# bartn8/vppstereo

Hardware: AMD Instinct MI355X
Metric: Mdisparities/s (HxWxD / s) VPP+rSGM at 540x960xD=192 (higher is better)
Workload: dtype u16

## Files before the change

### include/vppx.h

```cpp
#ifndef VPPX_H
#define VPPX_H

#include <stddef.h>
#include <stdint.h>

#ifdef __cplusplus
extern "C" {
#endif

#define VPPX_VERSION 100

enum {
    VPPX_OK = 0,
    VPPX_E_INVALID_ARG = -1,
    VPPX_E_DMAX_MOD8 = -2,
    VPPX_E_DMAX_GT256 = -3,
    VPPX_E_UNIQUENESS = -4,
    VPPX_E_WIDTH_MOD16 = -5,
    VPPX_E_METHOD = -6,
    VPPX_E_NO_DEVICE = -7,
    VPPX_E_HIP = -8,
    VPPX_E_OOM = -9,
    VPPX_E_UNSUPPORTED = -10
};
// ... 217 lines not shown
typedef struct vppx_fstream vppx_fstream;
int vppx_fstream_create(vppx_ctx *ctx, const VppxOccParams *op, const VppxVppParams *vp, const VppxRsgmParams *rp, int batch,
                        int depth, int H, int W, int C, int flags, int copy_threads, vppx_fstream **out);
void vppx_fstream_destroy(vppx_fstream *fs);
int vppx_fstream_create_scaled(vppx_ctx *ctx, const VppxOccParams *op, const VppxVppParams *vp, const VppxRsgmParams *rp,
                               const VppxScaleParams *sp, int batch, int depth, int H, int W, int C, int flags, int copy_threads,
                               vppx_fstream **out);

int vppx_fstream_push(vppx_fstream *fs, const uint8_t *left, const uint8_t *right, const float *hints, const uint8_t *g_occ);
int vppx_fstream_push_guided(vppx_fstream *fs, const uint8_t *left, const uint8_t *right, const float *hints, const uint8_t *g_occ,
                             const float *validhints);
int vppx_fstream_flush(vppx_fstream *fs);
int vppx_fstream_pop(vppx_fstream *fs, float *disp_out, uint8_t *l_vpp_out, uint8_t *r_vpp_out, uint8_t *conf_out,
                     uint64_t *draws_out, int *got);
int vppx_fstream_create_eval(vppx_ctx *ctx, const VppxOccParams *op, const VppxVppParams *vp, const VppxRsgmParams *rp,
                             const VppxScaleParams *sp, const VppxEvalParams *ep, int batch, int depth, int H, int W, int C, int flags,
                             int copy_threads, vppx_fstream **out);
int vppx_fstream_push_eval(vppx_fstream *fs, const uint8_t *left, const uint8_t *right, const float *hints, const uint8_t *g_occ,
                           const float *validhints, const float *gt, const float *validgt);
int vppx_fstream_pop_eval(vppx_fstream *fs, float *disp_out, uint8_t *l_vpp_out, uint8_t *r_vpp_out, uint8_t *conf_out,
                          uint64_t *draws_out, VppxMetrics *metrics_out, int *got);
int vppx_fstream_create_sampled(vppx_ctx *ctx, const VppxOccParams *op, const VppxVppParams *vp, const VppxRsgmParams *rp,
                                const VppxScaleParams *sp, const VppxEvalParams *ep, const VppxSampleParams *smp, int batch, int depth,
                                int H, int W, int C, int flags, int copy_threads, vppx_fstream **out);
int vppx_fstream_push_sampled(vppx_fstream *fs, const uint8_t *left, const uint8_t *right, const uint8_t *g_occ, const float *src,
                              const float *validsrc, const float *gt, const float *validgt);
int vppx_fstream_counts(vppx_fstream *fs, int64_t *pushed, int64_t *filling, int64_t *unpopped, int64_t *reruns);

int vppx_u8_to_nchw_dev(vppx_ctx *ctx, int B, int H, int W, int C, int pad_multiple, const uint8_t *src, void *dst,
                        int dst_is_bf16);

int vppx_psmnet_cost_volume_dev(vppx_ctx *ctx, const float *fea_l, const float *fea_r, const float *hints,
                                const float *validhints, int B, int C, int H4, int W4, int H, int W, int maxdisp,
                                float *cost);
int vppx_raft_corr_modulate_dev(vppx_ctx *ctx, float *corr, const float *hints, const float *validhints, int B, int H4,
                                int W2, int W3, int H, int W);
typedef enum VppxDtype {
    VPPX_DT_F32 = 0,
    VPPX_DT_BF16 = 1
} VppxDtype;
int vppx_psmnet_cost_volume_dt_dev(vppx_ctx *ctx, const void *fea_l, const void *fea_r, const float *hints,
                                   const float *validhints, int B, int C, int H4, int W4, int H, int W, int maxdisp,
                                   void *cost, int dtype);
int vppx_raft_corr_modulate_dt_dev(vppx_ctx *ctx, void *corr, const float *hints, const float *validhints, int B, int H4,
                                   int W2, int W3, int H, int W, int dtype);
#define VPPX_CORR_MAX_LEVELS 4
#define VPPX_CORR_MAX_RADIUS 8
int64_t vppx_raft_corr_pyramid_cells(int64_t N, int W3, int levels, int64_t *offsets);
int vppx_raft_corr_pyramid_dt_dev(vppx_ctx *ctx, void *corr, const float *hints, const float *validhints, int B, int H4, int W2,
                                  int W3, int H, int W, int levels, void *pyr, int dtype);
int vppx_raft_corr_lookup_dt_dev(vppx_ctx *ctx, const void *corr, const void *pyr, const float *coords_x,
                                 int64_t coords_frame_stride, int B, int H4, int W2, int W3, int levels, int radius,
                                 float *out, int dtype);
int vppx_psmnet_readout_dt_dev(vppx_ctx *ctx, const void *cost, int B, int D4, int H4, int W4, int maxdisp, int H, int W,
                               int top, int left, int Hout, int Wout, float *out, int dtype);
int vppx_raft_upsample_dt_dev(vppx_ctx *ctx, const void *flow, int64_t flow_frame_stride, const void *mask, int B, int C,
                              int H4, int W4, int f, int mask_channels, int sign, int top, int left, int Hout, int Wout,
                              float *out, int dtype);
int vppx_kitti_disp_decode_dev(vppx_ctx *ctx, const uint16_t *png_u16, int64_t n, float *disp, uint8_t *valid);
int vppx_png_decode_dev(vppx_ctx *ctx, int n_files, const uint8_t *blob, const int64_t *offsets, int H, int W, int C,
                        float scale, float *disp, uint8_t *valid, uint8_t *out_u8, int32_t *status);
int vppx_pfm_decode_dev(vppx_ctx *ctx, const uint8_t *raw, int H, int W, int channels, int little_endian, float *out);

int vppx_occlusion_heuristic_host(vppx_ctx *ctx, int B, int H, int W, const float *hints, int rx, int ry, double l,
                                  double g, double th_conf, double th_filter, uint8_t *conf_out);
int vppx_occlusion_heuristic_dev(vppx_ctx *ctx, int B, int H, int W, const float *hints, int rx, int ry, double l,
                                 double g, double th_conf, double th_filter, uint8_t *conf_out);
int vppx_occlusion_heuristic_full_host(vppx_ctx *ctx, int B, int H, int W, const float *hints, int rx, int ry, double l,
                                       double g, double th_conf, double th_filter, float *dmap_out, uint8_t *conf_out);
int vppx_occlusion_heuristic_full_dev(vppx_ctx *ctx, int B, int H, int W, const float *hints, int rx, int ry, double l,
                                      double g, double th_conf, double th_filter, float *dmap_out, uint8_t *conf_out);

int vppx_set_graph_mode(vppx_ctx *ctx, int enable);
long vppx_graph_replays(vppx_ctx *ctx);
int vppx_time_aggregate(vppx_ctx *ctx, int iters, float *ms_out);
int vppx_agg_kernel_ms(vppx_ctx *ctx, int last_n, float *avg_ms, int *n_used);
int vppx_we_kernel_ms(vppx_ctx *ctx, int last_n, float *avg_ms, int *n_used);
int vppx_time_aggregate_frames(vppx_ctx *ctx);
int vppx_time_aggregate_part(vppx_ctx *ctx, int iters, int part, float *ms_out);
int vppx_uses_vert(vppx_ctx *ctx);
int vppx_fused_pixels_per_wave(vppx_ctx *ctx);
int vppx_batch_quantum(vppx_ctx *ctx, int H, int W, int dmax);
int vppx_last_call_parts(vppx_ctx *ctx);
int vppx_we_last_pieces(vppx_ctx *ctx);
int vppx_wsum_last_pieces(vppx_ctx *ctx);
int vppx_wsum_default_route(int B, int Hp, int Wp, int dmax, int p2max, int nsimd);
int vppx_last_routes(vppx_ctx *ctx, char *buf, int n);
int vppx_last_front_routes(vppx_ctx *ctx, char *buf, int n);
int vppx_enable_stage_timing(vppx_ctx *ctx, int enable);
int vppx_get_stage_ms(vppx_ctx *ctx, float *ms, int max_n);
const char *vppx_stage_name(int i);


#ifdef __cplusplus
}
#endif
#endif
```

### vppstereo_amd/_lib.py

```python
import ctypes as C
import os
import threading

import numpy as np

_HERE = os.path.dirname(os.path.abspath(__file__))
LIB_PATH = os.environ.get("VPPX_LIB") or os.path.join(_HERE, "libvppx.so")

VPPX_OK = 0
ERR_NAMES = {
    -1: "VPPX_E_INVALID_ARG", -2: "VPPX_E_DMAX_MOD8", -3: "VPPX_E_DMAX_GT256", -4: "VPPX_E_UNIQUENESS",
    -5: "VPPX_E_WIDTH_MOD16", -6: "VPPX_E_METHOD", -7: "VPPX_E_NO_DEVICE", -8: "VPPX_E_HIP", -9: "VPPX_E_OOM",
    -10: "VPPX_E_UNSUPPORTED",
}

EXPORTS = [
    "vppx_version", "vppx_last_error", "vppx_vpp_params_default", "vppx_rsgm_params_default", "vppx_occ_params_default", "vppx_create",
    "vppx_destroy", "vppx_set_stream", "vppx_set_stream_legacy", "vppx_set_pipeline", "vppx_synchronize", "vppx_status", "vppx_lockstep_failures", "vppx_workspace_bytes", "vppx_device_name", "vppx_srand",
    "vppx_rand_stream", "vppx_rand_state", "vppx_rand_advance", "vppx_virtual_projection_scan_rnd", "vppx_virtual_projection_scan_max_dist", "vppx_vpp_host",
    "vppx_vpp_dev", "vppx_vpp_last_draws", "vppx_census5x5", "vppx_cost_census5x5_xyd", "vppx_aggregate", "vppx_aggregate_img", "vppx_match_wta",
    "vppx_match_wta_right", "vppx_subpixel_refine", "vppx_median3x3", "vppx_rsgm_host", "vppx_rsgm_dev",
    "vppx_vpp_rsgm_dev", "vppx_rsgm_post_dev", "vppx_occ_vpp_rsgm_dev", "vppx_occ_vpp_rsgm_host", "vppx_inputs_ready_event", "vppx_u8_to_nchw_dev", "vppx_psmnet_cost_volume_dev", "vppx_raft_corr_modulate_dev", "vppx_kitti_disp_decode_dev", "vppx_png_decode_dev", "vppx_pfm_decode_dev", "vppx_occlusion_heuristic_host", "vppx_occlusion_heuristic_dev", "vppx_occlusion_heuristic_full_host", "vppx_occlusion_heuristic_full_dev", "vppx_set_graph_mode", "vppx_graph_replays", "vppx_time_aggregate", "vppx_agg_kernel_ms", "vppx_we_kernel_ms", "vppx_time_aggregate_frames", "vppx_time_aggregate_part", "vppx_uses_vert", "vppx_last_call_parts", "vppx_we_last_pieces", "vppx_wsum_last_pieces", "vppx_wsum_default_route", "vppx_last_routes", "vppx_last_front_routes", "vppx_fused_pixels_per_wave", "vppx_batch_quantum",
    "vppx_enable_stage_timing", "vppx_get_stage_ms", "vppx_stage_name",
    "vppx_fstream_create", "vppx_fstream_destroy", "vppx_fstream_push", "vppx_fstream_flush", "vppx_fstream_pop", "vppx_fstream_counts",
    "vppx_occ_vpp_rsgm_guided_dev", "vppx_occ_vpp_rsgm_guided_host", "vppx_fstream_push_guided",
    "vppx_scale_params_default", "vppx_scaled_shape", "vppx_scale_table_builds", "vppx_last_front_sets", "vppx_occ_vpp_rsgm_scaled_dev", "vppx_occ_vpp_rsgm_scaled_host",
    "vppx_fstream_create_scaled",
    "vppx_eval_params_default", "vppx_guided_metrics_dev", "vppx_guided_metrics_host", "vppx_occ_vpp_rsgm_eval_dev",
    "vppx_fstream_create_eval", "vppx_fstream_push_eval", "vppx_fstream_pop_eval",
    "vppx_rsgm_front_dev", "vppx_rsgm_guided_rows_dev", "vppx_rsgm_mid_dev",
    "vppx_error_colors_dev", "vppx_error_colors_host", "vppx_guided_visualize_dev", "vppx_guided_visualize_host",
    "vppx_colorize_dev", "vppx_colorize_host", "vppx_finite_max_dev",
    "vppx_sample_params_default", "vppx_sample_threshold", "vppx_sample_hints_dev", "vppx_sample_hints_host", "vppx_occ_vpp_rsgm_sampled_dev",
    "vppx_fstream_create_sampled", "vppx_fstream_push_sampled",
    "vppx_psmnet_cost_volume_dt_dev", "vppx_raft_corr_modulate_dt_dev",
    "vppx_raft_corr_pyramid_cells", "vppx_raft_corr_pyramid_dt_dev", "vppx_raft_corr_lookup_dt_dev",
    "vppx_psmnet_readout_dt_dev", "vppx_raft_upsample_dt_dev",
]
CORR_MAX_LEVELS, CORR_MAX_RADIUS = 4, 8
DT_F32, DT_BF16 = 0, 1
FS_PATTERNS, FS_MASK, FS_GOCC, FS_GUIDED = 1, 2, 4, 8
FS_METRICS, FS_NO_DISP = 16, 32
FS_SAMPLE = 64
VIZ_KEYS = ('bad 1.0', 'bad 2.0', 'bad 3.0', 'bad 4.0', 'avgerr', 'rms')
VIZ_ALL = 63
VIZ_MAX_DILATION = 31
METRIC_KEYS = ('bad 1.0', 'bad 2.0', 'bad 3.0', 'bad 4.0', 'avgerr', 'rms')


class VppxVppParams(C.Structure):
    _fields_ = [
        ("method", C.c_int32), ("wsize", C.c_int32), ("wsize_agg_x", C.c_int32), ("wsize_agg_y", C.c_int32),
        ("direction", C.c_int32), ("uniform_color", C.c_int32), ("discard_occluded", C.c_int32),
        ("interpolate", C.c_int32), ("c", C.c_float), ("c_occ", C.c_float), ("use_distance_patch", C.c_int32),
        ("use_bilateral_patch", C.c_int32), ("distance_gamma", C.c_double), ("dmin", C.c_float), ("dmax", C.c_float),
        ("seed", C.c_uint32), ("per_frame_range", C.c_uint32), ("rand_offset", C.c_uint64),
        ("bilateral_o_xy", C.c_double), ("bilateral_o_i", C.c_double), ("bilateral_th", C.c_double),
    ]


class VppxRsgmParams(C.Structure):
    _fields_ = [
        ("dmax", C.c_int32), ("p1", C.c_int32), ("p2min", C.c_int32), ("alpha", C.c_float), ("gamma", C.c_int32),
        ("uniqueness", C.c_float), ("subpixel", C.c_int32), ("reserved0", C.c_int32),
    ]


class VppxOccParams(C.Structure):
    _fields_ = [("rx", C.c_int32), ("ry", C.c_int32), ("l", C.c_double), ("g", C.c_double), ("th_conf", C.c_double),
                ("th_filter", C.c_double)]


class VppxScaleParams(C.Structure):
    _fields_ = [("iscale", C.c_int32), ("oscale", C.c_int32)]


class VppxEvalParams(C.Structure):
    _fields_ = [("gt_scale", C.c_int32), ("reserved0", C.c_int32)]


class VppxSampleParams(C.Structure):
    _fields_ = [("probability", C.c_double), ("seed", C.c_uint32), ("reserved0", C.c_uint32), ("reserved1", C.c_uint64)]


class VppxMetrics(C.Structure):
    _fields_ = [("bad1", C.c_double), ("bad2", C.c_double), ("bad3", C.c_double), ("bad4", C.c_double), ("avgerr", C.c_double),
                ("rms", C.c_double), ("n_valid", C.c_double), ("reserved", C.c_double)]


class VppxError(Exception):

    def __init__(self, code, msg):
        super().__init__(msg)
        self.code = code


_lib = None
_lock = threading.Lock()


def load():
    global _lib
    with _lock:
        if _lib is not None:
            return _lib
# ... 13 lines not shown
        lib.vppx_device_name.restype = C.c_char_p
        lib.vppx_device_name.argtypes = [vp]
        lib.vppx_stage_name.restype = C.c_char_p
        lib.vppx_stage_name.argtypes = [C.c_int]
        lib.vppx_workspace_bytes.restype = C.c_size_t
        lib.vppx_workspace_bytes.argtypes = [vp]
        lib.vppx_create.argtypes = [C.POINTER(vp), C.c_int]
        lib.vppx_destroy.argtypes = [vp]
        lib.vppx_destroy.restype = None
        lib.vppx_set_stream.argtypes = [vp, vp]
        lib.vppx_set_stream_legacy.argtypes = [vp]
        lib.vppx_set_pipeline.argtypes = [vp, C.c_int]
        lib.vppx_synchronize.argtypes = [vp]
        lib.vppx_status.argtypes = [vp]
        lib.vppx_lockstep_failures.argtypes = [vp]
        lib.vppx_lockstep_failures.restype = C.c_long
        lib.vppx_srand.argtypes = [vp, C.c_uint32]
        lib.vppx_rand_state.argtypes = [vp, C.POINTER(C.c_uint32), C.POINTER(C.c_uint64)]
        lib.vppx_rand_advance.argtypes = [vp, C.c_uint64]
        lib.vppx_rand_stream.argtypes = [vp, C.c_uint32, C.c_uint64, C.c_int64, vp]
        i, f, d = C.c_int, C.c_float, C.c_double
        lib.vppx_virtual_projection_scan_rnd.argtypes = [vp, vp, vp, vp, i, i, i, i, i, i, f, f, vp, i, i]
        lib.vppx_virtual_projection_scan_max_dist.argtypes = [vp, vp, vp, vp, i, i, i, i, i, i, i, i, f, f, vp, i, i]
        pv, pr = C.POINTER(VppxVppParams), C.POINTER(VppxRsgmParams)
        lib.vppx_vpp_params_default.argtypes = [pv]
        lib.vppx_vpp_params_default.restype = None
        lib.vppx_rsgm_params_default.argtypes = [pr]
        lib.vppx_rsgm_params_default.restype = None
        lib.vppx_vpp_host.argtypes = [vp, pv, i, i, i, i, vp, vp, vp, vp, vp, vp]
        lib.vppx_vpp_dev.argtypes = [vp, pv, i, i, i, i, vp, vp, vp, vp, vp, vp]
        lib.vppx_vpp_last_draws.argtypes = [vp, i, C.POINTER(C.c_uint64)]
        lib.vppx_census5x5.argtypes = [vp, vp, vp, i, i]
        lib.vppx_cost_census5x5_xyd.argtypes = [vp, vp, vp, vp, i, i, i, i]
        lib.vppx_aggregate.argtypes = [vp, vp, vp, vp, i, i, i, i, i, f, i]
        lib.vppx_aggregate_img.argtypes = [vp, vp, i, vp, vp, i, i, i, i, i, f, i]
        lib.vppx_match_wta.argtypes = [vp, vp, vp, i, i, i, f]
        lib.vppx_match_wta_right.argtypes = [vp, vp, vp, i, i, i, f]
        lib.vppx_subpixel_refine.argtypes = [vp, vp, vp, i, i, i, i]
        lib.vppx_median3x3.argtypes = [vp, vp, vp, i, i]
        lib.vppx_rsgm_host.argtypes = [vp, pr, i, i, i, i, vp, vp, vp, vp, vp, vp]
        lib.vppx_rsgm_dev.argtypes = [vp, pr, i, i, i, i, vp, vp, vp, vp, vp, vp]
        lib.vppx_rsgm_post_dev.argtypes = [vp, i, i, i, vp, vp, i, vp]
        lib.vppx_rsgm_front_dev.argtypes = [vp, i, i, i, i, vp, vp, vp, vp, vp, vp]
        lib.vppx_rsgm_guided_rows_dev.argtypes = [vp, i, i, i, i, vp, vp, vp, vp, vp, vp, vp]
        lib.vppx_rsgm_mid_dev.argtypes = [vp, i, i, i, vp, vp, vp, vp]
        lib.vppx_vpp_rsgm_dev.argtypes = [vp, pv, pr, i, i, i, i, vp, vp, vp, vp, vp, vp, vp]
        po = C.POINTER(VppxOccParams)
        lib.vppx_occ_vpp_rsgm_host.argtypes = [vp, po, pv, pr, i, i, i, i, vp, vp, vp, vp, vp, vp, vp, vp, C.POINTER(C.c_uint64)]
        lib.vppx_occ_params_default.argtypes = [po]
        lib.vppx_occ_params_default.restype = None
        lib.vppx_occ_vpp_rsgm_dev.argtypes = [vp, po, pv, pr, i, i, i, i, vp, vp, vp, vp, vp, vp, vp]
        lib.vppx_occ_vpp_rsgm_guided_dev.argtypes = [vp, po, pv, pr, i, i, i, i, vp, vp, vp, vp, vp, vp, vp, vp, vp]
        lib.vppx_occ_vpp_rsgm_guided_host.argtypes = [vp, po, pv, pr, i, i, i, i, vp, vp, vp, vp, vp, vp, vp, vp, vp,
                                                      C.POINTER(C.c_uint64)]
        lib.vppx_inputs_ready_event.argtypes = [vp, vp]
        lib.vppx_u8_to_nchw_dev.argtypes = [vp, i, i, i, i, i, vp, vp, i]
        lib.vppx_psmnet_cost_volume_dev.argtypes = [vp, vp, vp, vp, vp, i, i, i, i, i, i, i, vp]
        lib.vppx_raft_corr_modulate_dev.argtypes = [vp, vp, vp, vp, i, i, i, i, i, i]
        lib.vppx_psmnet_cost_volume_dt_dev.argtypes = [vp, vp, vp, vp, vp, i, i, i, i, i, i, i, vp, i]
        lib.vppx_raft_corr_modulate_dt_dev.argtypes = [vp, vp, vp, vp, i, i, i, i, i, i, i]
        lib.vppx_raft_corr_pyramid_cells.argtypes = [C.c_int64, i, i, C.POINTER(C.c_int64)]
        lib.vppx_raft_corr_pyramid_cells.restype = C.c_int64
        lib.vppx_raft_corr_pyramid_dt_dev.argtypes = [vp, vp, vp, vp, i, i, i, i, i, i, i, vp, i]
        lib.vppx_raft_corr_lookup_dt_dev.argtypes = [vp, vp, vp, vp, C.c_int64, i, i, i, i, i, i, vp, i]
        lib.vppx_psmnet_readout_dt_dev.argtypes = [vp, vp, i, i, i, i, i, i, i, i, i, i, i, vp, i]
        lib.vppx_raft_upsample_dt_dev.argtypes = [vp, vp, C.c_int64, vp, i, i, i, i, i, i, i, i, i, i, i, vp, i]
        lib.vppx_kitti_disp_decode_dev.argtypes = [vp, vp, C.c_int64, vp, vp]
        lib.vppx_pfm_decode_dev.argtypes = [vp, vp, i, i, i, i, vp]
        lib.vppx_png_decode_dev.argtypes = [vp, i, vp, C.POINTER(C.c_int64), i, i, i, f, vp, vp, vp, vp]
        lib.vppx_occlusion_heuristic_host.argtypes = [vp, i, i, i, vp, i, i, d, d, d, d, vp]
        lib.vppx_occlusion_heuristic_dev.argtypes = [vp, i, i, i, vp, i, i, d, d, d, d, vp]
        lib.vppx_occlusion_heuristic_full_host.argtypes = [vp, i, i, i, vp, i, i, d, d, d, d, vp, vp]
        lib.vppx_occlusion_heuristic_full_dev.argtypes = [vp, i, i, i, vp, i, i, d, d, d, d, vp, vp]
        lib.vppx_set_graph_mode.argtypes = [vp, i]
        lib.vppx_graph_replays.argtypes = [vp]
        lib.vppx_graph_replays.restype = C.c_long
        lib.vppx_time_aggregate.argtypes = [vp, i, C.POINTER(C.c_float)]
        lib.vppx_agg_kernel_ms.argtypes = [vp, i, C.POINTER(C.c_float), C.POINTER(C.c_int)]
        lib.vppx_we_kernel_ms.argtypes = [vp, i, C.POINTER(C.c_float), C.POINTER(C.c_int)]
        lib.vppx_time_aggregate_frames.argtypes = [vp]
        lib.vppx_time_aggregate_part.argtypes = [vp, i, i, C.POINTER(C.c_float)]
        lib.vppx_uses_vert.argtypes = [vp]
        lib.vppx_last_call_parts.argtypes = [vp]
        lib.vppx_we_last_pieces.argtypes = [vp]
        lib.vppx_wsum_last_pieces.argtypes = [vp]
        lib.vppx_wsum_default_route.argtypes = [i, i, i, i, i, i]
        lib.vppx_last_routes.argtypes = [vp, C.c_char_p, i]
        lib.vppx_last_front_routes.argtypes = [vp, C.c_char_p, i]
        lib.vppx_fused_pixels_per_wave.argtypes = [vp]
        lib.vppx_batch_quantum.argtypes = [vp, i, i, i]
        lib.vppx_enable_stage_timing.argtypes = [vp, i]
        lib.vppx_get_stage_ms.argtypes = [vp, C.POINTER(C.c_float), i]
        lib.vppx_fstream_create.argtypes = [vp, po, pv, pr, i, i, i, i, i, i, i, C.POINTER(vp)]
        lib.vppx_fstream_destroy.argtypes = [vp]
        lib.vppx_fstream_destroy.restype = None
        lib.vppx_fstream_push.argtypes = [vp, vp, vp, vp, vp]
        lib.vppx_fstream_push_guided.argtypes = [vp, vp, vp, vp, vp, vp]
        lib.vppx_fstream_flush.argtypes = [vp]
        lib.vppx_fstream_pop.argtypes = [vp, vp, vp, vp, vp, C.POINTER(C.c_uint64), C.POINTER(C.c_int)]
        ps = C.POINTER(VppxScaleParams)
        lib.vppx_scale_params_default.argtypes = [ps]
        lib.vppx_scale_params_default.restype = None
        pi = C.POINTER(C.c_int)
        lib.vppx_scaled_shape.argtypes = [i, i, ps, pi, pi, pi, pi]
        lib.vppx_scale_table_builds.argtypes = [vp]
        lib.vppx_scale_table_builds.restype = C.c_long
        lib.vppx_last_front_sets.argtypes = [vp, pi, pi]
        lib.vppx_occ_vpp_rsgm_scaled_dev.argtypes = [vp, po, pv, pr, ps, i, i, i, i, vp, vp, vp, vp, vp, vp, vp, vp, vp, vp]
        lib.vppx_occ_vpp_rsgm_scaled_host.argtypes = [vp, po, pv, pr, ps, i, i, i, i, vp, vp, vp, vp, vp, vp, vp, vp, vp, vp,
                                                      C.POINTER(C.c_uint64)]
        lib.vppx_fstream_create_scaled.argtypes = [vp, po, pv, pr, ps, i, i, i, i, i, i, i, C.POINTER(vp)]
        p64 = C.POINTER(C.c_int64)
        lib.vppx_fstream_counts.argtypes = [vp, p64, p64, p64, p64]
        pe = C.POINTER(VppxEvalParams)
        lib.vppx_eval_params_default.argtypes = [pe]
        lib.vppx_eval_params_default.restype = None
        lib.vppx_guided_metrics_dev.argtypes = [vp, pe, i, i, i, vp, i, i, vp, vp, vp, vp]
        lib.vppx_guided_metrics_host.argtypes = [vp, pe, i, i, i, vp, i, i, vp, vp, vp, vp]
        lib.vppx_occ_vpp_rsgm_eval_dev.argtypes = [vp, po, pv, pr, ps, pe, i, i, i, i, vp, vp, vp, vp, vp, vp, vp, vp, vp, vp, vp, vp, vp, vp]
        lib.vppx_fstream_create_eval.argtypes = [vp, po, pv, pr, ps, pe, i, i, i, i, i, i, i, C.POINTER(vp)]
        lib.vppx_fstream_push_eval.argtypes = [vp, vp, vp, vp, vp, vp, vp, vp]
        lib.vppx_fstream_pop_eval.argtypes = [vp, vp, vp, vp, vp, C.POINTER(C.c_uint64), C.POINTER(VppxMetrics), C.POINTER(C.c_int)]
        u = C.c_uint
        for sfx in ("dev", "host"):
            getattr(lib, "vppx_error_colors_" + sfx).argtypes = [vp, i, i, i, vp, vp, d, i, i, vp]
            getattr(lib, "vppx_guided_visualize_" + sfx).argtypes = [vp, i, i, i, vp, vp, vp, d, i, u, vp]
            getattr(lib, "vppx_colorize_" + sfx).argtypes = [vp, i, i, i, vp, vp, vp, i, vp]
        lib.vppx_finite_max_dev.argtypes = [vp, i, i, i, vp, vp]
        pm = C.POINTER(VppxSampleParams)
        lib.vppx_sample_params_default.argtypes = [pm]
        lib.vppx_sample_params_default.restype = None
        lib.vppx_sample_threshold.argtypes = [d]
        lib.vppx_sample_threshold.restype = C.c_uint32
        lib.vppx_sample_hints_dev.argtypes = [vp, pm, i, i, i, vp, vp, vp, vp]
        lib.vppx_sample_hints_host.argtypes = [vp, pm, i, i, i, vp, vp, vp, vp]
        lib.vppx_occ_vpp_rsgm_sampled_dev.argtypes = [vp, po, pv, pr, ps, pe, pm, i, i, i, i, vp, vp, vp, vp, i, vp, vp, vp, vp, vp, vp, vp, vp,
                                                      vp, vp, vp, vp]
        lib.vppx_fstream_create_sampled.argtypes = [vp, po, pv, pr, ps, pe, pm, i, i, i, i, i, i, i, C.POINTER(vp)]
        lib.vppx_fstream_push_sampled.argtypes = [vp, vp, vp, vp, vp, vp, vp, vp]
        _lib = lib
        return lib


def split_routes(s):
    out, depth, cur = [], 0, []
    for ch in s:
        if ch == "," and depth == 0:
            out.append("".join(cur))
            cur = []
            continue
        depth += (ch == "<") - (ch == ">")
        cur.append(ch)
    if cur:
        out.append("".join(cur))
    return out


def _route_list(fn, handle):
    n = check(fn(handle, None, 0))
    buf = C.create_string_buffer(n + 1)
    check(fn(handle, buf, n + 1))
    return split_routes(buf.value.decode())


def last_routes(lib, handle):
    return _route_list(lib.vppx_last_routes, handle)
# ... 182 lines not shown
```

### vppstereo_amd/csrc/rsgm_kernels.hip

```cpp
#include "vppx_internal.h"

#include <stdlib.h>

#define INVALID_DISP_COST 16u
#define INVALID_DISP (-10.0f)

typedef u32 u32x4 __attribute__((ext_vector_type(4)));
typedef u32 u32x2 __attribute__((ext_vector_type(2)));
typedef u16 u16x2 __attribute__((ext_vector_type(2)));

__device__ __forceinline__ u32 pk_min(u32 a, u32 b)
{
    u16x2 r = __builtin_elementwise_min(__builtin_bit_cast(u16x2, a), __builtin_bit_cast(u16x2, b));
    return __builtin_bit_cast(u32, r);
}
__device__ __forceinline__ u32 pk_adds(u32 a, u32 b)
{
    u16x2 r = __builtin_elementwise_add_sat(__builtin_bit_cast(u16x2, a), __builtin_bit_cast(u16x2, b));
    return __builtin_bit_cast(u32, r);
}
__device__ __forceinline__ u32 pk_sub(u32 a, u32 b)
{
    u16x2 r = __builtin_bit_cast(u16x2, a) - __builtin_bit_cast(u16x2, b);
    return __builtin_bit_cast(u32, r);
// ... 2154 lines not shown
    ctx->v3.ok = pattern && nxcd == 8 && ctx->v3.cus_per_xcd > 0;
    *ok = ctx->v3.ok;
    return 0;
}

bool rsgm_vert3_supported(int B, int Hp, int Wp, int D, int maxp2)
{
    return (D == 64 || D == 128 || D == 192 || D == 256) && 3 * (24 + maxp2) <= 255 && B > 0 && Wp % 8 == 0 && Hp < 4095 &&
           (size_t)2 * B * (Wp / 8) * (V3_RING * 2 * 8 * 32) * sizeof(u32) < ((size_t)1 << 30);
}

static int v3_dk(int D) { return D == 64 ? 0 : (D == 128 ? 1 : (D == 192 ? 2 : 3)); }
static bool v3_wide(const vppx_ctx *ctx, int B, int Wp, int D)
{
    if (Wp % 16 != 0 || ctx->v3.ppw == 8) return false;
    if (ctx->v3.ppw == 16) return true;
    const int nbg = (Wp / 16 + 3) / 4;
    const int resident = ctx->v3.cus_per_xcd * ctx->v3.blocks_per_cu16[v3_dk(D)] / (nbg > 0 ? nbg : 1);
    return resident > 0 && (2 * B + 7) / 8 >= resident;
}

bool rsgm_vert3_wide(const vppx_ctx *ctx, int B, int Wp, int D) { return v3_wide(ctx, B, Wp, D); }

int rsgm_vert3_frames_per_round(const vppx_ctx *ctx, int Wp, int D)
{
    if (!ctx->v3.ok || Wp % 16 != 0 || !(D == 64 || D == 128 || D == 192 || D == 256)) return 0;
    const int nbg = (Wp / 16 + 3) / 4;
    const int resident = ctx->v3.cus_per_xcd * ctx->v3.blocks_per_cu16[v3_dk(D)] / nbg;
    return resident * ctx->v3.nxcd / 2;
}

bool rsgm_vert3_fits(const vppx_ctx *ctx, int B, int Wp, int D)
{
    if (!ctx->v3.ok) return false;
    const int k = v3_dk(D);
    const bool wide = v3_wide(ctx, B, Wp, D);
    const int nwv = wide ? Wp / 16 : Wp / 8;
    const int nbg = (nwv + 3) / 4;
    const int bpc = wide ? ctx->v3.blocks_per_cu16[k] : ctx->v3.blocks_per_cu[k];
    return nbg <= ctx->v3.cus_per_xcd * bpc * 3 / 4;
}
static int v3_rec_dwords(bool wide, int D)
{
    if (!wide) return V3_RING * 2 * 8 * (D == 256 ? V3Rec<16>::XW : 16);
    return V3_RING * 2 * 4 * (D == 64 ? V3Rec<8>::XW : (D == 128 ? V3Rec<16>::XW : (D == 192 ? V3Rec<24>::XW : V3Rec<32>::XW)));
}
size_t rsgm_vert3_xbuf_bytes(int B, int Wp, int D)
{
    const size_t narrow = (size_t)2 * B * (Wp / 8) * v3_rec_dwords(false, D);
    const size_t wide = (size_t)2 * B * (Wp / 16) * v3_rec_dwords(true, D);
    return ((narrow > wide ? narrow : wide) + 128) * sizeof(u32);
}
static size_t v3_xbuf_bytes_one(int B, int Wp, int D)
{
    const size_t narrow = (size_t)2 * B * (Wp / 8) * v3_rec_dwords(false, D);
    const size_t wide = (size_t)2 * B * (Wp / 16) * v3_rec_dwords(true, D);
    return ((narrow > wide ? narrow : wide) + 64) * sizeof(u32);
}

void rsgm_vert3_plan(const vppx_ctx *ctx, int B, int Wp, int D, int *whole_frames, bool *rest_underfilled)
{
    *whole_frames = 0;
    *rest_underfilled = false;
    const int fpr = rsgm_vert3_frames_per_round(ctx, Wp, D);
    if (fpr <= 0 || !ctx->v3.ok) return;
    int rest = B;
    if (v3_wide(ctx, B, Wp, D) && B > fpr && B % fpr != 0) {
        *whole_frames = B - B % fpr;
        rest = B % fpr;
    } else if (B >= fpr) {
        return;
    }
    *rest_underfilled = 3 * rest <= 2 * fpr;
}

int rsgm_launch_vert3_range(vppx_ctx *ctx, hipStream_t stream, int B_total, int f0, int nB, int Hp, int Wp, int D, const u8 *gray,
                            const u32 *cl, const u32 *cr, const u16 *p2lut, int p1, u8 *sv, u32 *xbuf, unsigned *err, unsigned *err_dev,
                            bool next_to_we)
{
    if (f0 == 0) {
        ++ctx->v3.serial;
        if (ctx->v3.serial == 0) ++ctx->v3.serial;
        const size_t xbytes = rsgm_vert3_xbuf_bytes(B_total, Wp, D);
        if (!(ctx->xbuf_cleared && !ctx->capturing && ctx->xbuf_last == (void *)xbuf && ctx->xbuf_last_bytes >= xbytes && stream == ctx->stream))
            VPPX_HIP(hipMemsetAsync(xbuf, 0, xbytes, stream));
        ctx->xbuf_last = (void *)xbuf;
        ctx->xbuf_last_bytes = xbytes;
        ctx->xbuf_cleared = false;
    } else {
        xbuf += v3_xbuf_bytes_one(f0, Wp, D) / sizeof(u32);
    }
    const size_t fpix = (size_t)f0 * Hp * Wp;
    Vert3Args a;
    a.gray = gray + fpix; a.cl = cl + fpix; a.cr = cr + fpix; a.p2lut = p2lut; a.sv = sv + fpix * D; a.xbuf = xbuf; a.err = err; a.err_dev = err_dev;
    a.B = nB; a.Hp = Hp; a.Wp = Wp;
    a.p1 = p1 > 231 ? 231 : p1;
    bool wide = v3_wide(ctx, nB, Wp, D);
    if (!wide && next_to_we && Wp % 16 == 0 && ctx->v3.ppw == 0) {
        const int nbg16 = (Wp / 16 + 3) / 4;
        const int resident = ctx->v3.cus_per_xcd * ctx->v3.blocks_per_cu16[v3_dk(D)] / (nbg16 > 0 ? nbg16 : 1);
        wide = resident >= 4 && 2 * nB >= ctx->v3.nxcd * ((resident + 1) / 2);
    }
    {
        const int k = v3_dk(D);
        auto fits = [&](bool w) {
            const int nbg = ((w ? Wp / 16 : Wp / 8) + 3) / 4;
            const int bpc = w ? ctx->v3.blocks_per_cu16[k] : ctx->v3.blocks_per_cu[k];
            return (!w || Wp % 16 == 0) && nbg <= ctx->v3.cus_per_xcd * bpc * 3 / 4;
        };
        if (!fits(wide) && fits(!wide)) wide = !wide;
    }
    if (f0 == 0) ctx->v3.last_ppw = wide ? 16 : 8;
    a.nwv = wide ? Wp / 16 : Wp / 8;
    a.nbg = (a.nwv + 3) / 4;
    a.vol_elems = (size_t)B_total * Hp * Wp * D;
    a.timeout_ticks = (long long)ctx->v3.timeout_ms * (long long)(ctx->v3.wall_khz > 0 ? ctx->v3.wall_khz : 100000);
    a.spin_limit = ctx->v3.spin_limit;
    a.serial = ctx->v3.serial;
    const dim3 grid((unsigned)((2 * nB + 7) / 8 * 8 * a.nbg));
    if (wide && D == 64) sgm_vert4_kernel<16><<<grid, 256, 0, stream>>>(a);
    else if (wide && D == 128) sgm_vert4_kernel<32><<<grid, 256, 0, stream>>>(a);
    else if (wide && D == 192) sgm_vert4_kernel<48><<<grid, 256, 0, stream>>>(a);
    else if (wide) sgm_vert4_kernel<64><<<grid, 256, 0, stream>>>(a);
    else if (D == 64) sgm_vert3_kernel<8><<<grid, 256, 0, stream>>>(a);
    else if (D == 128) sgm_vert3_kernel<16><<<grid, 256, 0, stream>>>(a);
    else if (D == 192) sgm_vert3_kernel<24><<<grid, 256, 0, stream>>>(a);
    else sgm_vert3_kernel<32><<<grid, 256, 0, stream>>>(a);
    VPPX_CHECK_LAUNCH();
    route_note(ctx, wide ? "vert4<%d>" : "vert3<%d>", (wide ? D / 4 : D / 8));
    return 0;
}

int rsgm_launch_vert3(vppx_ctx *ctx, hipStream_t stream, int B, int Hp, int Wp, int D, const u8 *gray, const u32 *cl,
                      const u32 *cr, const u16 *p2lut, int p1, u8 *sv, u32 *xbuf, unsigned *err, unsigned *err_dev)
{
    return rsgm_launch_vert3_range(ctx, stream, B, 0, B, Hp, Wp, D, gray, cl, cr, p2lut, p1, sv, xbuf, err, err_dev, false);
}

template <int DPL>
__device__ __forceinline__ float wta_rows(const u32 (&S)[DPL / 2], int dbase, int n , int D,
                                          u32 factor_uniq, bool do_subpixel, bool x_interior)
{
    constexpr int NP = DPL / 2;
    u32 key = 0xFFFFFFFFu;
#pragma unroll
    for (int i = 0; i < NP; i++) {
        const int d0 = dbase + 2 * i, d1 = d0 + 1;
        const u32 k0 = d0 < n ? (((S[i] & 0xFFFFu) << 8) | (u32)d0) : 0xFFFFFFFFu;
        const u32 k1 = d1 < n ? (((S[i] >> 16) << 8) | (u32)d1) : 0xFFFFFFFFu;
        key = min(key, min(k0, k1));
    }
    key = row_min_u32(key);
    const int best = (int)(key & 0xFFu);
    const u32 minc = key >> 8;
    u32 sec = 65535u, cm1 = 0, cp1 = 0, nbhit = 0;
#pragma unroll
    for (int i = 0; i < NP; i++) {
        const int d0 = dbase + 2 * i, d1 = d0 + 1;
        const u32 s0 = S[i] & 0xFFFFu, s1 = S[i] >> 16;
        if (d0 < n && d0 != best) sec = min(sec, s0);
        if (d1 < n && d1 != best) sec = min(sec, s1);
        if (d0 == best - 1) cm1 = s0;
        if (d1 == best - 1) cm1 = s1;
        if (d0 == best + 1) cp1 = s0;
        if (d1 == best + 1) cp1 = s1;
    }
    sec = row_min_u32(sec);
// ... 1762 lines not shown
            sub[u] = dlr[x];
        }
#pragma unroll
        for (int u = 0; u < 4; u++) r2[u] = lb[r1[u]];
#pragma unroll
        for (int u = 0; u < 4; u++) {
            int r = r1[u], pr = r2[u];
            while (pr != r) {
                r = pr;
                pr = lb[r];
            }
            r1[u] = r;
        }
        int sz[4];
#pragma unroll
        for (int u = 0; u < 4; u++) sz[u] = size[base + r1[u]];
#pragma unroll
        for (int u = 0; u < 4; u++) {
            const int x = xb + 256 * u;
            int vv = v[u];
            if (vv != new_val && sz[u] <= max_size) vv = new_val;
            float fv = (float)vv;
            if (subpixel && fv != 0.0f) fv = sub[u];
            if (x < W) val[x] = fv;
        }
    }
    __syncthreads();
    const int SEG = (W + 255) / 256;
    const int x0 = threadIdx.x * SEG;
    int lastv = -1, firstv = 0x7FFFFFFF;
    for (int j = 0; j < SEG; j++) {
        const int x = x0 + j;
        if (x < W && val[x] > 0) {
            lastv = x;
            if (firstv == 0x7FFFFFFF) firstv = x;
        }
    }
    int sl = lastv, sr = firstv;
#pragma unroll
    for (int off = 1; off < 64; off <<= 1) {
        const int tl = __shfl_up(sl, off), tr = __shfl_down(sr, off);
        if (lane >= off) sl = max(sl, tl);
        if (lane + off < 64) sr = min(sr, tr);
    }
    if (lane == 63) s_l[wv] = sl;
    if (lane == 0) s_r[wv] = sr;
    __syncthreads();
    if (threadIdx.x == 0) row_any[(size_t)f * H + y] = max(max(s_l[0], s_l[1]), max(s_l[2], s_l[3])) >= 0 ? 1 : 0;
    int cl = __shfl_up(sl, 1), cr = __shfl_down(sr, 1);
    if (lane == 0) cl = -1;
    if (lane == 63) cr = 0x7FFFFFFF;
    for (int w = 0; w < wv; w++) cl = max(cl, s_l[w]);
    for (int w = wv + 1; w < 4; w++) cr = min(cr, s_r[w]);
    int xl[SEGMAX];
#pragma unroll
    for (int j = 0; j < SEGMAX; j++) {
        const int x = x0 + j;
        if (j < SEG && x < W && val[x] > 0) cl = x;
        xl[j] = cl;
    }
#pragma unroll
    for (int j = SEGMAX - 1; j >= 0; j--) {
        const int x = x0 + j;
        if (j >= SEG || x >= W) continue;
        float v = val[x];
        if (v > 0) {
            cr = x;
        } else {
            const bool hl = xl[j] >= 0, hr = cr < W;
            if (hl && hr) {
                const float a = val[xl[j]], b = val[cr];
                v = b < a ? b : a;
            } else if (hr) {
                v = val[cr];
            } else if (hl) {
                v = val[xl[j]];
            }
        }
        res[x] = v;
    }
    __syncthreads();
    for (int x = threadIdx.x; x < W; x += 256) g[x] = res[x];
}
__global__ void __launch_bounds__(256) interp_bg_edge_rows_kernel(float *__restrict__ dm, const u8 *__restrict__ row_any, int H, int W)
{
    __shared__ int s_first[4], s_last[4];
    const int f = blockIdx.x, lane = threadIdx.x & 63, wv = threadIdx.x >> 6;
    float *g = dm + (size_t)f * H * W;
    int first = 0x7FFFFFFF, last = -1;
    for (int v = threadIdx.x; v < H; v += 256)
        if (row_any[(size_t)f * H + v]) { first = min(first, v); last = max(last, v); }
#pragma unroll
    for (int off = 32; off >= 1; off >>= 1) {
        first = min(first, __shfl_xor(first, off));
        last = max(last, __shfl_xor(last, off));
    }
    if (lane == 0) s_first[wv] = first, s_last[wv] = last;
    __syncthreads();
    first = min(min(s_first[0], s_first[1]), min(s_first[2], s_first[3]));
    last = max(max(s_last[0], s_last[1]), max(s_last[2], s_last[3]));
    if (last < 0) return;
    for (size_t i = threadIdx.x; i < (size_t)first * W; i += 256) g[i] = g[(size_t)first * W + i % W];
    for (size_t i = (size_t)(last + 1) * W + threadIdx.x; i < (size_t)H * W; i += 256) g[i] = g[(size_t)last * W + i % W];
}

__global__ void __launch_bounds__(256) void_if_lost_kernel(float *__restrict__ out, size_t n, const unsigned *__restrict__ err_dev,
                                                           unsigned serial)
{
    if (__hip_atomic_load(err_dev, __ATOMIC_RELAXED, __HIP_MEMORY_SCOPE_AGENT) != serial) return;
    const float nan = __builtin_nanf("");
    for (size_t i = (size_t)blockIdx.x * 256 + threadIdx.x; i < n; i += (size_t)gridDim.x * 256) out[i] = nan;
}

int rsgm_launch_void_if_lost(vppx_ctx *ctx, float *out, size_t n, const unsigned *err_dev, unsigned serial)
{
    const unsigned nblk = (unsigned)((n + 256 * 16 - 1) / (256 * 16));
    void_if_lost_kernel<<<nblk < 1 ? 1 : nblk, 256, 0, ctx->stream>>>(out, n, err_dev, serial);
    VPPX_CHECK_LAUNCH();
    return 0;
}

int rsgm_launch_post(vppx_ctx *ctx, const RsgmGeom &g, const float *dl_pad, const float *dr_pad, int subpixel, float *out)
{
    const size_t n = (size_t)g.B * g.H * g.W, npf = (size_t)g.H * g.W;
    if (g.W > 8192) { vppx_set_error("frame width %d > 8192 is not supported by the post-processing kernels", g.W); return VPPX_E_UNSUPPORTED; }
    const int ntx = (g.W + SPK_TW - 1) / SPK_TW, nty = (g.H + SPK_TH - 1) / SPK_TH;
    const size_t ntiles = (size_t)ntx * nty * g.B;
    u8 *fd8, *row_any;
    int *label, *size, *roots, *nroots;
    int rc;
    if ((rc = ws_get(ctx, WS_FD8, n, &fd8))) return rc;
    if ((rc = ws_get(ctx, WS_LABEL, n, &label))) return rc;
    if ((rc = ws_get(ctx, WS_LCOUNT, n, &size))) return rc;
    if ((rc = ws_get(ctx, WS_SPK_ROOTS, ntiles * (SPK_TW * SPK_TH), &roots))) return rc;
    if ((rc = ws_get(ctx, WS_SPK_NROOTS, ntiles, &nroots))) return rc;
    if ((rc = ws_get(ctx, WS_ROW_ANY, (size_t)g.B * g.H, &row_any))) return rc;
    speckle_tile_kernel<<<dim3(ntx, nty, g.B), 256, 0, ctx->stream>>>(dl_pad, dr_pad, fd8, label, size, roots, nroots, g.H, g.W, g.Hp, g.Wp,
                                                                      g.pad_t, g.pad_l, 0, 10);
    VPPX_CHECK_LAUNCH();
    const int nby = (g.H - 1) / SPK_TH, nbx = (g.W - 1) / SPK_TW;
    const int nlinks = nby * g.W + nbx * g.H;
    if (nlinks > 0) {
        speckle_border_kernel<<<dim3((nlinks + 255) / 256, g.B), 256, 0, ctx->stream>>>(fd8, label, g.H, g.W, 0, 10);
        VPPX_CHECK_LAUNCH();
    }
    speckle_total_kernel<<<(unsigned)ntiles, 64, 0, ctx->stream>>>(label, size, roots, nroots, npf, ntx * nty);
    VPPX_CHECK_LAUNCH();
    const size_t lds = (size_t)g.W * 2 * sizeof(float);
    if (g.W <= 2048)
        speckle_apply_rows_kernel<8><<<dim3(g.H, g.B), 256, lds, ctx->stream>>>(fd8, label, size, dl_pad, out, row_any, g.H, g.W, g.Hp, g.Wp,
                                                                               g.pad_t, g.pad_l, 0, 200, subpixel);
    else
        speckle_apply_rows_kernel<32><<<dim3(g.H, g.B), 256, lds, ctx->stream>>>(fd8, label, size, dl_pad, out, row_any, g.H, g.W, g.Hp, g.Wp,
                                                                                g.pad_t, g.pad_l, 0, 200, subpixel);
    VPPX_CHECK_LAUNCH();
    interp_bg_edge_rows_kernel<<<g.B, 256, 0, ctx->stream>>>(out, row_any, g.H, g.W);
    VPPX_CHECK_LAUNCH();
    return 0;
}
```

### vppstereo_amd/csrc/vppx_api.hip

```cpp
#include "vppx_internal.h"

#include <limits.h>
#include <math.h>
#include <stdarg.h>
#include <stdlib.h>
#include <string.h>

static thread_local char g_err[1024] = "";

void vppx_set_error(const char *fmt, ...)
{
    va_list ap;
    va_start(ap, fmt);
    vsnprintf(g_err, sizeof(g_err), fmt, ap);
    va_end(ap);
}

extern "C" const char *vppx_last_error(void) { return g_err; }

static void note_once(std::vector<std::string> &list, const char *name)
{
    for (const std::string &r : list)
        if (r == name) return;
    list.emplace_back(name);
// ... 119 lines not shown
        }
        b.cap = cap;
        ctx->total_bytes += cap;
    }
    *out = b.p;
    return 0;
}

extern "C" int vppx_create(vppx_ctx **out, int device)
{
    if (!out) { vppx_set_error("vppx_create: out is NULL"); return VPPX_E_INVALID_ARG; }
    *out = nullptr;
    int ndev = 0;
    hipError_t e = hipGetDeviceCount(&ndev);
    if (e != hipSuccess || ndev <= 0) {
        vppx_set_error("no HIP device available (%s); libvppx has no CPU fallback",
                       e != hipSuccess ? hipGetErrorString(e) : "device count is 0");
        return VPPX_E_NO_DEVICE;
    }
    if (device < 0) {
        if (hipGetDevice(&device) != hipSuccess) device = 0;
    }
    if (device >= ndev) { vppx_set_error("device %d out of range (%d devices)", device, ndev); return VPPX_E_INVALID_ARG; }
    DevGuard dev_guard_(device);
    vppx_ctx *ctx = new vppx_ctx();
    ctx->device = device;
    hipDeviceProp_t prop;
    if (hipGetDeviceProperties(&prop, device) == hipSuccess) {
        ctx->devname = prop.name[0] ? prop.name : prop.gcnArchName;
        if (strstr(prop.gcnArchName, "gfx950") == nullptr) {
            vppx_set_error("device %d is %s; libvppx is built for gfx950 only", device, prop.gcnArchName);
            delete ctx;
            return VPPX_E_NO_DEVICE;
        }
    }
    e = hipStreamCreateWithFlags(&ctx->stream, hipStreamNonBlocking);
    if (e != hipSuccess) {
        vppx_set_error("hipStreamCreate failed: %s", hipGetErrorString(e));
        delete ctx;
        return VPPX_E_HIP;
    }
    ctx->own_stream = true;
    if (hipStreamCreateWithFlags(&ctx->stream2, hipStreamNonBlocking) != hipSuccess ||
        hipEventCreateWithFlags(&ctx->ev_fork, hipEventDisableTiming) != hipSuccess ||
        hipEventCreateWithFlags(&ctx->ev_join, hipEventDisableTiming) != hipSuccess) {
        vppx_set_error("side stream / event creation failed");
        delete ctx;
        return VPPX_E_HIP;
    }
    {
        const char *e = getenv("VPPX_VERT");
        ctx->use_vert = e ? atoi(e) : -1;
        e = getenv("VPPX_CHUNK");
        if (e) ctx->knobs.chunk = atoi(e);
        e = getenv("VPPX_VARIANT");
        if (e) {
            std::string v(e);
            auto has = [&](const char *tok) { return ("," + v + ",").find(std::string(",") + tok + ",") != std::string::npos; };
            if (has("sum_general")) ctx->knobs.sum_general = 1;
            if (has("gw4")) ctx->knobs.gw = 4;
            if (has("gw8")) ctx->knobs.gw = 8;
            if (has("gw16")) ctx->knobs.gw = 16;
            if (has("maxdist_lds")) ctx->knobs.maxdist = 1;
            if (has("maxdist_global")) ctx->knobs.maxdist = 2;
            if (has("we_line")) ctx->knobs.we_line = 1;
            if (has("sum_gl8")) ctx->knobs.sum_gl8 = 1;
            if (has("sum_trap0")) ctx->knobs.sum_trap = 0;
            if (has("sum_trap1")) ctx->knobs.sum_trap = 1;
            if (has("we_after")) ctx->knobs.we_next = 0;
            if (has("we_whole")) ctx->knobs.we_split = 0;
            if (has("we_mute")) ctx->knobs.we_mute = 1;
            if (has("we_stale")) ctx->knobs.we_stale = 1;
            {
                const size_t fk = v.find("fs_fail_submit="), ff = v.find("fs_fail_from=");
                if (fk != std::string::npos) ctx->knobs.fs_fail_submit = atoi(v.c_str() + fk + 15);
                if (ff != std::string::npos) ctx->knobs.fs_fail_from = atoi(v.c_str() + ff + 13);
            }
            {
                const size_t wl = v.find("we_layer=");
                if (wl != std::string::npos) ctx->knobs.we_layer = atoi(v.c_str() + wl + 9);
            }
            if (has("wsum")) ctx->knobs.wsum = 1;
            if (has("nowsum")) ctx->knobs.wsum = 0;
            {
                const size_t wc = v.find("wsum_cut=");
                if (wc != std::string::npos) ctx->knobs.wsum_cut = atoi(v.c_str() + wc + 9);
            }
            if (has("we_lq0")) ctx->knobs.we_lq = 0;
            if (has("we_lq1")) ctx->knobs.we_lq = 1;
#ifdef VPPX_EXPERIMENT
            if (has("pipe_mid")) ctx->pipe_mid = true;
            const size_t sb = v.find("sum_blocks=");
            if (sb != std::string::npos) ctx->knobs.sum_blocks = atoi(v.c_str() + sb + 11);
#endif
        }
        e = getenv("VPPX_SUBSTREAMS");
        if (e) ctx->nsub = atoi(e) < 1 ? 1 : (atoi(e) > 4 ? 4 : atoi(e));
        e = getenv("VPPX_V3_TIMEOUT_MS");
        if (e && atoi(e) > 0) ctx->v3.timeout_ms = atoi(e);
        e = getenv("VPPX_V3_PPW");
        if (e && (atoi(e) == 8 || atoi(e) == 16)) ctx->v3.ppw = atoi(e);
#ifdef VPPX_EXPERIMENT
        e = getenv("VPPX_V3_IGNORE_LOST");
        if (e && atoi(e) > 0) ctx->v3.ignore_lost = true;
        e = getenv("VPPX_EXP_WE_TRACE");
        if (e && *e) ctx->exp_we_trace = e;
#endif
        e = getenv("VPPX_V3_SPIN_LIMIT");
        if (e && atoi(e) > 0) ctx->v3.spin_limit = (unsigned)atoi(e);
        e = getenv("VPPX_GUIDED_PART_MB");
        if (e && atoll(e) > 0) ctx->knobs.guided_part_bytes = (unsigned long long)atoll(e) << 20;
    }
    *out = ctx;
    return 0;
}

extern "C" void vppx_destroy(vppx_ctx *ctx)
{
    if (!ctx) return;
    DevGuard dev_guard_(ctx->device);
    (void)hipDeviceSynchronize();
    for (int i = 0; i < 4; i++) {
        if (ctx->sub[i]) vppx_destroy(ctx->sub[i]);
        if (ctx->sub_done[i]) (void)hipEventDestroy(ctx->sub_done[i]);
    }
    for (int i = 0; i < WS_NUM; i++)
        if (ctx->ws[i].p) (void)hipFree(ctx->ws[i].p);
    if (ctx->ev_created)
        for (int i = 0; i <= VPPX_MAX_STAGES; i++) (void)hipEventDestroy(ctx->ev[i]);
    if (ctx->gexec) (void)hipGraphExecDestroy(ctx->gexec);
    if (ctx->agg_ev_created)
        for (int j = 0; j < 2; j++)
            for (int i = 0; i < vppx_ctx::AGG_RING; i++) {
                (void)hipEventDestroy(ctx->agg_ev[j][i]);
                (void)hipEventDestroy(ctx->we_ev[j][i]);
            }
    if (ctx->own_stream && ctx->stream) (void)hipStreamDestroy(ctx->stream);
    if (ctx->vert3_err) (void)hipHostFree(ctx->vert3_err);
    if (ctx->stream_front) (void)hipStreamDestroy(ctx->stream_front);
    if (ctx->ev_agg_done) (void)hipEventDestroy(ctx->ev_agg_done);
    if (ctx->ev_front_done) (void)hipEventDestroy(ctx->ev_front_done);
    if (ctx->ev_occ_done) (void)hipEventDestroy(ctx->ev_occ_done);
    if (ctx->ev_inputs_auto) (void)hipEventDestroy(ctx->ev_inputs_auto);
    if (ctx->ev_scaled) (void)hipEventDestroy(ctx->ev_scaled);
    if (ctx->ev_sampled) (void)hipEventDestroy(ctx->ev_sampled);
    if (ctx->stream2) (void)hipStreamDestroy(ctx->stream2);
    if (ctx->ev_fork) (void)hipEventDestroy(ctx->ev_fork);
    if (ctx->ev_join) (void)hipEventDestroy(ctx->ev_join);
    delete ctx;
}

extern "C" int vppx_set_graph_mode(vppx_ctx *ctx, int enable)
{
    if (!ctx) return VPPX_E_INVALID_ARG;
    ctx->graph_mode = enable != 0;
    if (!enable && ctx->gexec) { (void)hipGraphExecDestroy(ctx->gexec); ctx->gexec = nullptr; ctx->have_gkey = false; }
    ctx->have_lastkey = false;
    return 0;
}

extern "C" long vppx_graph_replays(vppx_ctx *ctx) { return ctx ? ctx->graph_replays : 0; }
extern "C" long vppx_scale_table_builds(vppx_ctx *ctx) { return ctx ? ctx->scale_tab_builds : 0; }
extern "C" int vppx_last_front_sets(vppx_ctx *ctx, int *scale_set, int *sample_set)
{
    if (!ctx) { vppx_set_error("vppx_last_front_sets: ctx is NULL"); return VPPX_E_INVALID_ARG; }
    if (scale_set) *scale_set = ctx->last_scale_set;
    if (sample_set) *sample_set = ctx->last_sample_set;
    return 0;
}

static int release_own_stream(vppx_ctx *ctx)
{
    if (ctx->own_stream && ctx->stream) {
        VPPX_HIP(hipStreamSynchronize(ctx->stream));
        (void)hipStreamDestroy(ctx->stream);
    }
    ctx->own_stream = false;
    ctx->stream = nullptr;
    return 0;
}

extern "C" int vppx_set_stream(vppx_ctx *ctx, void *hip_stream)
{
    VPPX_ENTER(ctx);
    if (hip_stream != nullptr) {
        if (ctx->stream == (hipStream_t)hip_stream && !ctx->own_stream && !ctx->legacy_stream) {
            VPPX_PIPE_KEEP(ctx);
            return 0;
        }
        int rc = release_own_stream(ctx);
        if (rc) return rc;
        ctx->stream = (hipStream_t)hip_stream;
        ctx->legacy_stream = false;
    } else if (!ctx->own_stream) {
        VPPX_HIP(hipStreamCreateWithFlags(&ctx->stream, hipStreamNonBlocking));
        ctx->own_stream = true;
        ctx->legacy_stream = false;
    }
    return 0;
}

extern "C" int vppx_set_stream_legacy(vppx_ctx *ctx)
{
    VPPX_ENTER(ctx);
    if (ctx->legacy_stream) {
        VPPX_PIPE_KEEP(ctx);
        return 0;
    }
    int rc = release_own_stream(ctx);
    if (rc) return rc;
    ctx->stream = nullptr;
    ctx->legacy_stream = true;
    return 0;
}

static int lockstep_check(vppx_ctx *ctx)
{
    if (!ctx->vert3_err || !ctx->vert3_err[0]) return 0;
    const unsigned serial = ctx->vert3_err[0];
    ctx->vert3_err[0] = 0;
    ctx->lockstep_failures++;
    ctx->lockstep_last_serial = serial;
    if (ctx->v3.ignore_lost) return 0;
    ctx->vert3_rest = ctx->vert3_backoff;
    ctx->vert3_backoff = ctx->vert3_backoff < 4096 ? ctx->vert3_backoff * 2 : 4096;
    if (ctx->gexec) {
        (void)hipGraphExecDestroy(ctx->gexec);
        ctx->gexec = nullptr;
        ctx->have_gkey = false;
    }
    ctx->have_lastkey = false;
    vppx_set_error("fused aggregation launch #%u lost its lock step (a wave waited longer than %d ms%s for its neighbour): the "
                   "disparities of that call are void, and so are those of fused calls queued behind it (last launch: #%u); "
                   "the context uses the line-parallel aggregation kernel for its next %d aggregation launches, then tries the fused layout again",
                   serial, ctx->v3.timeout_ms, ctx->v3.spin_limit ? " / VPPX_V3_SPIN_LIMIT polls" : "", ctx->v3.serial, ctx->vert3_rest);
    return VPPX_E_HIP;
}

int vppx_lockstep_check_internal(vppx_ctx *ctx) { return lockstep_check(ctx); }
static int check_frames(int B, int H, int W, int C);
static int check_vpp_params(const VppxVppParams &p);
static int check_rsgm_params(const VppxRsgmParams &p);
int vppx_check_hot_path_args_internal(const VppxVppParams *vp, const VppxRsgmParams *rp, int B, int H, int W, int C)
{
    int rc;
    if ((rc = check_frames(B, H, W, C))) return rc;
    if ((rc = check_vpp_params(*vp))) return rc;
    return check_rsgm_params(*rp);
}

extern "C" int vppx_synchronize(vppx_ctx *ctx)
{
    VPPX_ENTER(ctx);
    VPPX_HIP(hipStreamSynchronize(ctx->stream));
    return lockstep_check(ctx);
}

extern "C" int vppx_status(vppx_ctx *ctx)
{
    VPPX_ENTER(ctx);
    VPPX_PIPE_KEEP(ctx);
    return lockstep_check(ctx);
}

extern "C" long vppx_lockstep_failures(vppx_ctx *ctx) { return ctx ? ctx->lockstep_failures : 0; }
extern "C" int vppx_fused_pixels_per_wave(vppx_ctx *ctx) { return (ctx && ctx->last_vert == 3) ? ctx->v3.last_ppw : 0; }

static void make_geom(int B, int H, int W, int C, int D, RsgmGeom &g);
static int v3_probe_once(vppx_ctx *ctx);
extern "C" int vppx_batch_quantum(vppx_ctx *ctx, int H, int W, int dmax)
{
    if (!ctx || H < 1 || W < 1 || ctx->capturing) return 0;
    DevGuard dev_guard_(ctx->device);
    if (ctx->vert3_broken || v3_probe_once(ctx) != 0 || ctx->vert3_broken) return 0;
    RsgmGeom g;
    make_geom(1, H, W, 3, dmax, g);
    return rsgm_vert3_frames_per_round(ctx, g.Wp, g.D);
}

extern "C" size_t vppx_workspace_bytes(const vppx_ctx *ctx)
{
    if (!ctx) return 0;
    size_t t = ctx->total_bytes;
    for (int i = 0; i < 4; i++)
        if (ctx->sub[i]) t += ctx->sub[i]->total_bytes;
    return t;
}
extern "C" const char *vppx_device_name(const vppx_ctx *ctx) { return ctx ? ctx->devname.c_str() : ""; }

static const char *k_stage_names[ST_COUNT] = {"vpp_compact", "vpp_rand", "vpp_apply", "pad_gray", "census",
                                              "aggregate_8paths", "sum_wta_left", "wta_right", "median_interp", "post",
                                              "occlusion_heuristic"};

extern "C" const char *vppx_stage_name(int i) { return (i >= 0 && i < ST_COUNT) ? k_stage_names[i] : ""; }

// ... 189 lines not shown
    VPPX_HIP(hipMemcpy(host, g_exp_trace_buf, (size_t)g_exp_trace_n * 16, hipMemcpyDeviceToHost));
    return 0;
}
static int exp_env(const char *name)
{
    const char *e = getenv(name);
    return e ? atoi(e) : 0;
}
static int exp_pre_we(vppx_ctx *ctx, const RsgmGeom &g, const u8 *gl, const u32 *cl, const u32 *cr, void *paths, size_t ncell)
{
    const int mode = exp_env("VPPX_EXP_PRE");
    u32 *sink = (u32 *)ctx->ws[WS_P2LUT].p + 200;
    const size_t npp = (size_t)g.B * g.Hp * g.Wp;
    if (mode == 1) {
        exp_read_kernel<<<2048, 256, 0, ctx->stream>>>((const uint4 *)cl, npp / 4, 1, sink);
        exp_read_kernel<<<2048, 256, 0, ctx->stream>>>((const uint4 *)cr, npp / 4, 1, sink);
        exp_read_kernel<<<2048, 256, 0, ctx->stream>>>((const uint4 *)gl, npp / 16, 1, sink);
    } else if (mode == 2) {
        exp_read_kernel<<<2048, 256, 0, ctx->stream>>>((const uint4 *)paths, ncell * 2 / 4096, 256, sink);
    } else if (mode == 3) {
        exp_spin_kernel<<<4096, 256, 0, ctx->stream>>>(sink, 20000);
    } else if (mode == 6) {
        exp_write_kernel<<<2048, 256, 0, ctx->stream>>>((u32 *)paths, ncell * 2 / 4096, 1024);
    }
    VPPX_CHECK_LAUNCH();
    return 0;
}
#endif

static int agg_events_create(vppx_ctx *ctx)
{
    if (ctx->agg_ev_created) return 0;
    for (int j = 0; j < 2; j++)
        for (int i = 0; i < vppx_ctx::AGG_RING; i++) {
            VPPX_HIP(hipEventCreate(&ctx->agg_ev[j][i]));
            VPPX_HIP(hipEventCreate(&ctx->we_ev[j][i]));
        }
    ctx->agg_ev_created = true;
    return 0;
}

static int run_aggregation(vppx_ctx *ctx, const VppxRsgmParams &p, const RsgmGeom &g, const u8 *gl, const u32 *cl,
                           const u32 *cr, const u16 *lut_d, int maxp2, const void **vols, int *nvol_out,
                           int *elem_bytes_out, int which, const float *hints = nullptr, const float *validhints = nullptr)
{
    int rc;
    const size_t npp = (size_t)g.B * g.Hp * g.Wp;
    const size_t ncell = npp * g.D;
    int nvol;
    ctx->wsum_route = false;
    if ((rc = lockstep_check(ctx))) return rc;
    if (hints && validhints) {
        u16 *rows;
        int *gmap;
        void *gp;
        if ((rc = ws_get(ctx, WS_DSI, (size_t)g.B * g.H * g.W * g.D, &rows))) return rc;
        if ((rc = ws_get(ctx, WS_GUIDED_MAP, npp + 1, &gmap))) return rc;
        if ((rc = ws_reserve(ctx, WS_PATHS, ncell * 8 * 2, &gp))) return rc;
        if ((rc = rsgm_launch_guided_rows(ctx, g, cl, cr, hints, validhints, gmap, rows, (u32 *)(gmap + npp)))) return rc;
        if ((rc = rsgm_launch_paths(ctx, g.B, g.Hp, g.Wp, g.D, gl, cl, cr, rows, lut_d, p.p1, gp, 2, 0xFF, gmap))) return rc;
        for (int k = 0; k < 8; k++) vols[k] = (const u8 *)gp + (size_t)k * ncell * 2;
        *nvol_out = 8;
        *elem_bytes_out = 2;
        return 0;
    }
    const int elem_bytes = rsgm_paths_elem_bytes(g.D, maxp2);
    bool vert3;
    if ((rc = fused_layout_wanted(ctx, g, maxp2, &vert3))) return rc;
    if (!vert3 && ctx->vert3_rest > 0 && which == 0) ctx->vert3_rest--;
    const bool vert = vert3 || (ctx->use_vert == 1 && elem_bytes == 1 && rsgm_vert_supported(g.D, maxp2) && g.D <= 192);
    ctx->last_vert = vert3 ? 3 : (vert ? 1 : 0);
    void *paths;
    if (vert) {
        u8 *sv, *gst;
        u16 *gmin;
        if ((rc = ws_reserve(ctx, WS_PATHS, ncell * 2, &paths))) return rc;
        if ((rc = ws_get(ctx, WS_SV, ncell * 2, &sv))) return rc;
        if ((rc = ws_get(ctx, WS_VSTATE, vert3 ? rsgm_vert3_xbuf_bytes(g.B, g.Wp, g.D) : rsgm_vert_state_bytes(g.B, g.Wp, g.D), &gst))) return rc;
        if ((rc = ws_get(ctx, WS_VMIN, vert3 ? 8 : rsgm_vert_min_elems(g.B, g.Wp), &gmin))) return rc;
        ctx->wsum_route = vert3 && elem_bytes == 1 && rsgm_wsum_eligible(ctx, g.B, g.Hp, g.Wp, g.D, maxp2, rsgm_device_simds(ctx));
        const int we_dirs = ctx->wsum_route ? 0x10 : 0x11;
        bool we_launched = false;
        auto launch_we = [&]() -> int {
            const bool timed = !ctx->capturing;
            if (timed && (rc = agg_events_create(ctx))) return rc;
            const int slot = (int)(ctx->we_calls % vppx_ctx::AGG_RING);
#ifdef VPPX_EXPERIMENT
            if ((rc = exp_pre_we(ctx, g, gl, cl, cr, paths, ncell))) return rc;
            if (exp_env("VPPX_EXP_TWICE") && (rc = rsgm_launch_paths(ctx, g.B, g.Hp, g.Wp, g.D, gl, cl, cr, nullptr, lut_d, p.p1, paths, 1, 0x11))) return rc;
#endif
            if (timed) VPPX_HIP(hipEventRecord(ctx->we_ev[0][slot], ctx->stream));
            const int r = rsgm_launch_paths(ctx, g.B, g.Hp, g.Wp, g.D, gl, cl, cr, nullptr, lut_d, p.p1, paths, 1, we_dirs);
            if (timed) {
                VPPX_HIP(hipEventRecord(ctx->we_ev[1][slot], ctx->stream));
                ctx->we_calls++;
            }
            return r;
        };
        auto launch_vert = [&](hipStream_t st) -> int {
            if (!vert3) return rsgm_launch_vert(ctx, st, g.B, g.Hp, g.Wp, g.D, gl, cl, cr, lut_d, p.p1, sv, gst, gmin);
            if (!ctx->vert3_err) {
                if (hipHostMalloc((void **)&ctx->vert3_err, 64, hipHostMallocMapped) != hipSuccess) {
                    ctx->vert3_err = nullptr;
                    (void)hipGetLastError();
                    vppx_set_error("could not allocate the pinned status word of the fused aggregation kernel");
                    return VPPX_E_HIP;
                }
                ctx->vert3_err[0] = 0;
            }
            const bool timed = !ctx->capturing && st == ctx->stream;
            if (timed && (rc = agg_events_create(ctx))) return rc;
            const int slot = (int)(ctx->agg_calls % vppx_ctx::AGG_RING);
            if (timed) VPPX_HIP(hipEventRecord(ctx->agg_ev[0][slot], st));
            unsigned *err_dev;
            {
                const bool fresh = ctx->ws[WS_V3ERR].p == nullptr;
                if ((rc = ws_get(ctx, WS_V3ERR, (size_t)4, &err_dev))) return rc;
                if (fresh) VPPX_HIP(hipMemsetAsync(err_dev, 0, 16, st));
            }
            int whole = 0;
            bool rest_under = false;
            if (which == 0 && ctx->knobs.we_next && st == ctx->stream && !we_launched) rsgm_vert3_plan(ctx, g.B, g.Wp, g.D, &whole, &rest_under);
            int r;
            if (!rest_under) {
                r = rsgm_launch_vert3(ctx, st, g.B, g.Hp, g.Wp, g.D, gl, cl, cr, lut_d, p.p1, sv, (u32 *)gst, ctx->vert3_err, err_dev);
            } else {
                if (whole > 0 &&
                    (r = rsgm_launch_vert3_range(ctx, st, g.B, 0, whole, g.Hp, g.Wp, g.D, gl, cl, cr, lut_d, p.p1, sv, (u32 *)gst, ctx->vert3_err, err_dev, false))) return r;
                VPPX_HIP(hipEventRecord(ctx->ev_fork, st));
                VPPX_HIP(hipStreamWaitEvent(ctx->stream2, ctx->ev_fork, 0));
                ctx->stream = ctx->stream2;
                ctx->we_beside_vert = true;
                r = launch_we();
                ctx->we_beside_vert = false;
                ctx->stream = st;
                if (r) return r;
                VPPX_HIP(hipEventRecord(ctx->ev_join, ctx->stream2));
                r = rsgm_launch_vert3_range(ctx, st, g.B, whole, g.B - whole, g.Hp, g.Wp, g.D, gl, cl, cr, lut_d, p.p1, sv, (u32 *)gst, ctx->vert3_err, err_dev, true);
                if (timed) {
                    VPPX_HIP(hipEventRecord(ctx->agg_ev[1][slot], st));
                    ctx->agg_calls++;
                }
                VPPX_HIP(hipStreamWaitEvent(st, ctx->ev_join, 0));
                we_launched = true;
                return r;
            }
            if (timed) {
                VPPX_HIP(hipEventRecord(ctx->agg_ev[1][slot], st));
                ctx->agg_calls++;
            }
            return r;
        };
        if (which == 0 && vert3) {
#ifdef VPPX_EXPERIMENT
            const bool we_first = exp_env("VPPX_EXP_ORDER") != 0;
#else
            const bool we_first = false;
#endif
            if (we_first) {
                if ((rc = launch_we())) return rc;
                we_launched = true;
                if ((rc = launch_vert(ctx->stream))) return rc;
            } else {
                if ((rc = launch_vert(ctx->stream))) return rc;
                if (ctx->pipe_call && !ctx->pipe_early && ctx->pipe_mid) {
                    VPPX_HIP(hipEventRecord(ctx->ev_agg_done, ctx->stream));
                    ctx->have_agg_done = true;
                    ctx->agg_done_recorded = true;
                }
                if (!we_launched && (rc = launch_we())) return rc;
            }
        } else if (which == 0) {
            VPPX_HIP(hipEventRecord(ctx->ev_fork, ctx->stream));
            VPPX_HIP(hipStreamWaitEvent(ctx->stream2, ctx->ev_fork, 0));
            hipStream_t main_stream = ctx->stream;
            ctx->stream = ctx->stream2;
            rc = rsgm_launch_paths(ctx, g.B, g.Hp, g.Wp, g.D, gl, cl, cr, nullptr, lut_d, p.p1, paths, 1, 0x11);
            ctx->stream = main_stream;
            if (rc) return rc;
            VPPX_HIP(hipEventRecord(ctx->ev_join, ctx->stream2));
            if ((rc = launch_vert(ctx->stream))) return rc;
            VPPX_HIP(hipStreamWaitEvent(ctx->stream, ctx->ev_join, 0));
        } else if (which == 1) {
            if ((rc = launch_we())) return rc;
        } else {
            if ((rc = launch_vert(ctx->stream))) return rc;
        }
        vols[0] = paths;
        vols[1] = (const u8 *)paths + ncell;
        vols[2] = sv;
        vols[3] = sv + ncell;
        nvol = 4;
    } else {
        if ((rc = ws_reserve(ctx, WS_PATHS, ncell * 8 * elem_bytes, &paths))) return rc;
        if ((rc = agg_events_create(ctx))) return rc;
        if (ctx->capturing) {
            if ((rc = rsgm_launch_paths(ctx, g.B, g.Hp, g.Wp, g.D, gl, cl, cr, nullptr, lut_d, p.p1, paths, elem_bytes, 0xFF))) return rc;
        } else {
            const int slot = (int)(ctx->agg_calls % vppx_ctx::AGG_RING);
            VPPX_HIP(hipEventRecord(ctx->agg_ev[0][slot], ctx->stream));
            if ((rc = rsgm_launch_paths(ctx, g.B, g.Hp, g.Wp, g.D, gl, cl, cr, nullptr, lut_d, p.p1, paths, elem_bytes, 0xFF))) return rc;
            VPPX_HIP(hipEventRecord(ctx->agg_ev[1][slot], ctx->stream));
            ctx->agg_calls++;
        }
        for (int k = 0; k < 8; k++) vols[k] = (const u8 *)paths + (size_t)k * ncell * elem_bytes;
        nvol = 8;
    }
    *nvol_out = nvol;
    *elem_bytes_out = elem_bytes;
    return 0;
}

static bool pipeline_applies(const vppx_ctx *ctx)
{
    return ctx->pipeline && !ctx->capturing && !ctx->stage_timing && !ctx->is_child && !ctx->graph_mode && ctx->nsub <= 1;
}
static int front_begin(vppx_ctx *ctx)
{
    if (!ctx->stream_front) {
        VPPX_HIP(hipStreamCreateWithFlags(&ctx->stream_front, hipStreamNonBlocking));
        VPPX_HIP(hipEventCreateWithFlags(&ctx->ev_agg_done, hipEventDisableTiming));
        VPPX_HIP(hipEventCreateWithFlags(&ctx->ev_front_done, hipEventDisableTiming));
        VPPX_HIP(hipEventCreateWithFlags(&ctx->ev_inputs_auto, hipEventDisableTiming));
    }
    if (!ctx->have_agg_done) {
        VPPX_HIP(hipEventRecord(ctx->ev_agg_done, ctx->stream));
        ctx->have_agg_done = true;
        VPPX_HIP(hipStreamWaitEvent(ctx->stream_front, ctx->ev_agg_done, 0));
        if (ctx->inputs_ev) VPPX_HIP(hipStreamWaitEvent(ctx->stream_front, (hipEvent_t)ctx->inputs_ev, 0));
    } else {
        VPPX_HIP(hipStreamWaitEvent(ctx->stream_front, ctx->ev_agg_done, 0));
        if (ctx->inputs_ev) {
            VPPX_HIP(hipStreamWaitEvent(ctx->stream_front, (hipEvent_t)ctx->inputs_ev, 0));
        } else {
            VPPX_HIP(hipEventRecord(ctx->ev_inputs_auto, ctx->stream));
            VPPX_HIP(hipStreamWaitEvent(ctx->stream_front, ctx->ev_inputs_auto, 0));
        }
    }
    ctx->inputs_ev = nullptr;
    ctx->main_saved = ctx->stream;
    ctx->stream = ctx->stream_front;
    ctx->front_active = true;
    return 0;
}
static int front_end(vppx_ctx *ctx)
{
    if (!ctx->front_active) return 0;
    hipStream_t front = ctx->stream;
    ctx->stream = ctx->main_saved;
    ctx->front_active = false;
    VPPX_HIP(hipEventRecord(ctx->ev_front_done, front));
    if (ctx->xbuf_last && !ctx->xbuf_cleared && ctx->xbuf_last == ctx->ws[WS_VSTATE].p) {
        VPPX_HIP(hipMemsetAsync(ctx->xbuf_last, 0, ctx->xbuf_last_bytes, ctx->stream));
        ctx->xbuf_cleared = true;
    }
    if (ctx->occ_done_recorded) {
        bool any = false;
        for (int i = 0; i < ctx->n_pipe_copy; i++) any = any || ctx->pipe_copy[i].early;
        if (any) VPPX_HIP(hipStreamWaitEvent(ctx->stream, ctx->ev_occ_done, 0));
        for (int i = 0; i < ctx->n_pipe_copy; i++)
            if (ctx->pipe_copy[i].early)
                VPPX_HIP(hipMemcpyAsync(ctx->pipe_copy[i].dst, ctx->pipe_copy[i].src, ctx->pipe_copy[i].bytes, hipMemcpyDeviceToDevice, ctx->stream));
    }
    VPPX_HIP(hipStreamWaitEvent(ctx->stream, ctx->ev_front_done, 0));
    for (int i = 0; i < ctx->n_pipe_copy; i++)
        if (!(ctx->occ_done_recorded && ctx->pipe_copy[i].early))
            VPPX_HIP(hipMemcpyAsync(ctx->pipe_copy[i].dst, ctx->pipe_copy[i].src, ctx->pipe_copy[i].bytes, hipMemcpyDeviceToDevice, ctx->stream));
    ctx->n_pipe_copy = 0;
    ctx->occ_done_recorded = false;
    if (ctx->pipe_call && ctx->pipe_early) {
        VPPX_HIP(hipEventRecord(ctx->ev_agg_done, ctx->stream));
        ctx->have_agg_done = true;
    }
    return 0;
}
struct FrontGuard {
    vppx_ctx *ctx;
    ~FrontGuard()
    {
        if (ctx->front_active) {
            ctx->stream = ctx->main_saved;
            ctx->front_active = false;
        }
        ctx->pipe_call = false;
        ctx->n_pipe_copy = 0;
        ctx->occ_done_recorded = false;
    }
};

static int rsgm_core(vppx_ctx *ctx, const VppxRsgmParams &p, const RsgmGeom &g, const u8 *left, const u8 *left_vpp,
                     const u8 *right_vpp, float *disp_out, const float *hints = nullptr, const float *validhints = nullptr)
{
    int rc;
    const size_t npp = (size_t)g.B * g.Hp * g.Wp;
    const size_t ncell = npp * g.D;
    u8 *gl;
    u32 *cl, *cr_raw;
    const bool alt = ctx->pipe_call && (ctx->pipe_parity & 1);
    if (ctx->pipe_call) ctx->pipe_parity ^= 1;
    {
        bool fused = false;
        if (ctx->pipe_call && g.B < 8) {
            u16 lut_tmp[256];
            int mp2 = 0;
            p2_lut_host(p, lut_tmp, &mp2);
            if ((rc = fused_layout_wanted(ctx, g, mp2, &fused))) return rc;
        }
        ctx->pipe_early = ctx->pipe_call && g.B < 8 && !fused;
    }
    if ((rc = ws_get(ctx, alt ? WS_GRAY_L2 : WS_GRAY_L, npp, &gl))) return rc;
    if ((rc = ws_get(ctx, alt ? WS_CENSUS_L2 : WS_CENSUS_L, npp, &cl))) return rc;
    if ((rc = ws_get(ctx, alt ? WS_CENSUS_R2 : WS_CENSUS_R, npp + 512, &cr_raw))) return rc;
    u32 *cr = cr_raw + 512;
    ctx->last_gl = gl; ctx->last_cl = cl; ctx->last_cr = cr;
    if ((rc = rsgm_launch_pad_gray_census(ctx, g, left, left_vpp, right_vpp, gl, cl, cr))) return rc;
    stage_mark(ctx, ST_PAD_GRAY);
    stage_mark(ctx, ST_CENSUS);
    if ((rc = front_end(ctx))) return rc;

    u16 *lut_d;
    if ((rc = ws_get(ctx, WS_P2LUT, 256, &lut_d))) return rc;
    if (!ctx->lut_valid || ctx->lut_p2min != p.p2min || ctx->lut_gamma != p.gamma || ctx->lut_alpha != p.alpha) {
        if (ctx->capturing) { vppx_set_error("penalty table changed during graph capture"); return VPPX_E_HIP; }
        p2_lut_host(p, ctx->lut_host, &ctx->lut_maxp2);
        VPPX_HIP(hipMemcpyAsync(lut_d, ctx->lut_host, sizeof(ctx->lut_host), hipMemcpyHostToDevice, ctx->stream));
        ctx->lut_p2min = p.p2min; ctx->lut_gamma = p.gamma; ctx->lut_alpha = p.alpha;
        ctx->lut_valid = true;
    }
    const int maxp2 = ctx->lut_maxp2;
    const void *vols[8];
    int nvol = 0, elem_bytes = 1;
    ctx->agg_done_recorded = false;
    if ((rc = run_aggregation(ctx, p, g, gl, cl, cr, lut_d, maxp2, vols, &nvol, &elem_bytes, 0, hints, validhints))) return rc;
    if (ctx->pipe_call && !ctx->pipe_early && !ctx->agg_done_recorded) {
        VPPX_HIP(hipEventRecord(ctx->ev_agg_done, ctx->stream));
        ctx->have_agg_done = true;
    }
    stage_mark(ctx, ST_AGGREGATE);
    ctx->last_B = g.B; ctx->last_Hp = g.Hp; ctx->last_Wp = g.Wp; ctx->last_D = g.D; ctx->last_rp = p; ctx->have_last = true;

    float *dl0, *dl1, *dr0, *dr1;
    if ((rc = ws_get(ctx, WS_DISP_L0, npp, &dl0))) return rc;
    if ((rc = ws_get(ctx, WS_DISP_L1, npp, &dl1))) return rc;
    if ((rc = ws_get(ctx, WS_DISP_R0, npp, &dr0))) return rc;
    if ((rc = ws_get(ctx, WS_DISP_R1, npp, &dr1))) return rc;
    const u32 fu = uniq_factor(p.uniqueness);
    if (ctx->wsum_route)
        rc = rsgm_launch_wsum(ctx, g.B, g.Hp, g.Wp, g.D, gl, cl, cr, lut_d, p.p1, vols[1], vols[2], vols[3], dl0, dr0, fu);
    else
        rc = rsgm_launch_sum_wta_lr(ctx, g.B, g.Hp, g.Wp, g.D, vols, nvol, elem_bytes, dl0, dr0, fu, 1,
                                    (hints && validhints) ? 0 : 24 + maxp2);
    if (rc < 0) return rc;
    if (rc == 0) {
        stage_mark(ctx, ST_SUM_WTA);
        ctx->last_sum_nvol = nvol; ctx->last_sum_D = g.D; ctx->last_sum_B = g.B;
    } else {
        ctx->last_sum_nvol = 0;
        u16 *S;
        if ((rc = ws_get(ctx, WS_S, ncell, &S))) return rc;
        if ((rc = rsgm_launch_sum_wta(ctx, g.B, g.Hp, g.Wp, g.D, vols[0], elem_bytes, nullptr, S, dl0, fu, 1))) return rc;
        stage_mark(ctx, ST_SUM_WTA);
        if ((rc = rsgm_launch_wta_right_t(ctx, g.B, g.Hp, g.Wp, g.D, S, dr0, fu))) return rc;
        stage_mark(ctx, ST_WTA_RIGHT);
    }
    if ((rc = rsgm_launch_median_interp_clip(ctx, g.B, g.Hp, g.Wp, dl0, dl1, dr0, dr1))) return rc;
    stage_mark(ctx, ST_MEDIAN_INTERP);
    { float *t = dl0; dl0 = dl1; dl1 = t; t = dr0; dr0 = dr1; dr1 = t; }

    const size_t np = (size_t)g.B * g.H * g.W;
    if ((rc = rsgm_launch_post(ctx, g, dl0, dr0, p.subpixel, disp_out))) return rc;
    if (ctx->last_vert == 3 && ctx->ws[WS_V3ERR].p &&
        (rc = rsgm_launch_void_if_lost(ctx, disp_out, np, (const unsigned *)ctx->ws[WS_V3ERR].p, ctx->v3.serial))) return rc;
    stage_mark(ctx, ST_POST);
    return 0;
}

static int check_frames(int B, int H, int W, int C)
{
    if (B <= 0 || H <= 0 || W <= 0) { vppx_set_error("bad shape B=%d H=%d W=%d", B, H, W); return VPPX_E_INVALID_ARG; }
    if (C != 1 && C != 3) { vppx_set_error("channels must be 1 or 3 (got %d)", C); return VPPX_E_INVALID_ARG; }
    if (H < 5 || W < 5) { vppx_set_error("frame too small (%dx%d)", H, W); return VPPX_E_INVALID_ARG; }
    return 0;
}

static int guided_frames_per_part(const vppx_ctx *ctx, int H, int W, int C, int dmax)
{
    RsgmGeom g1;
    make_geom(1, H, W, C, dmax, g1);
    const unsigned long long per = (unsigned long long)g1.Hp * g1.Wp * g1.D * 16ull;
    const unsigned long long n = ctx->knobs.guided_part_bytes / per;
    return n < 1 ? 1 : (n > (unsigned long long)INT_MAX ? INT_MAX : (int)n);
}

extern "C" int vppx_rsgm_dev(vppx_ctx *ctx, const VppxRsgmParams *p, int B, int H, int W, int C, const uint8_t *left,
                             const uint8_t *left_vpp, const uint8_t *right_vpp, const float *hints,
                             const float *validhints, float *disp_out)
{
    int rc;
    VPPX_ENTER(ctx);
    routes_reset(ctx);
    if ((rc = lockstep_check(ctx))) return rc;
    if (!p || !left || !left_vpp || !right_vpp || !disp_out) { vppx_set_error("vppx_rsgm: NULL argument"); return VPPX_E_INVALID_ARG; }
    if ((rc = check_frames(B, H, W, C))) return rc;
    if ((rc = check_rsgm_params(*p))) return rc;
    if ((hints == nullptr) != (validhints == nullptr)) { hints = nullptr; validhints = nullptr; }
    RsgmGeom g;
    stage_begin(ctx);
    const int q = hints ? guided_frames_per_part(ctx, H, W, C, p->dmax) : B;
    if (q >= B) {
        make_geom(B, H, W, C, p->dmax, g);
        return rsgm_core(ctx, *p, g, left, left_vpp, right_vpp, disp_out, hints, validhints);
    }
    const size_t fpx = (size_t)H * W;
    for (int lo = 0; lo < B; lo += q) {
        const int nb = B - lo < q ? B - lo : q;
        make_geom(nb, H, W, C, p->dmax, g);
        ctx->stage_append = lo > 0;
        rc = rsgm_core(ctx, *p, g, left + (size_t)lo * fpx * C, left_vpp + (size_t)lo * fpx * C, right_vpp + (size_t)lo * fpx * C,
                       disp_out + (size_t)lo * fpx, hints + (size_t)lo * fpx, validhints + (size_t)lo * fpx);
        ctx->stage_append = false;
        if (rc) return rc;
    }
    return 0;
}

extern "C" int vppx_rsgm_post_dev(vppx_ctx *ctx, int B, int H, int W, const float *disp_l_pad, const float *disp_r_pad,
                                  int subpixel, float *disp_out)
{
    int rc;
    VPPX_ENTER(ctx);
    if (!disp_l_pad || !disp_r_pad || !disp_out) { vppx_set_error("vppx_rsgm_post: NULL argument"); return VPPX_E_INVALID_ARG; }
    if ((rc = check_frames(B, H, W, 1))) return rc;
    RsgmGeom g;
    make_geom(B, H, W, 1, 64, g);
    return rsgm_launch_post(ctx, g, disp_l_pad, disp_r_pad, subpixel, disp_out);
}

extern "C" int vppx_rsgm_front_dev(vppx_ctx *ctx, int B, int H, int W, int C, const uint8_t *left, const uint8_t *left_vpp,
                                   const uint8_t *right_vpp, uint8_t *gray_left, uint32_t *census_l, uint32_t *census_r)
{
    int rc;
    VPPX_ENTER(ctx);
    if (!left || !left_vpp || !right_vpp || !gray_left || !census_l || !census_r) {
        vppx_set_error("vppx_rsgm_front: NULL argument");
        return VPPX_E_INVALID_ARG;
    }
    if ((rc = check_frames(B, H, W, C))) return rc;
    RsgmGeom g;
    make_geom(B, H, W, C, 64, g);
    return rsgm_launch_pad_gray_census(ctx, g, left, left_vpp, right_vpp, gray_left, census_l, census_r);
}

extern "C" int vppx_rsgm_guided_rows_dev(vppx_ctx *ctx, int B, int H, int W, int dmax, const uint32_t *census_l,
                                         const uint32_t *census_r, const float *hints, const float *validhints, int32_t *gmap,
                                         uint16_t *rows, uint32_t *count)
// ... 141 lines not shown
    if (!ctx) { vppx_set_error("context is NULL"); return VPPX_E_NO_DEVICE; }
    if (seed) *seed = ctx->rnd_seed;
    if (consumed) *consumed = ctx->rnd_consumed;
    return 0;
}

extern "C" int vppx_rand_advance(vppx_ctx *ctx, uint64_t draws)
{
    if (!ctx) { vppx_set_error("context is NULL"); return VPPX_E_NO_DEVICE; }
    ctx->rnd_consumed += draws;
    return 0;
}

static int scan_common(vppx_ctx *ctx, VppxVppParams &p, uint8_t *l, uint8_t *r, const float *g, int width, int height,
                       int channels, const uint8_t *g_occ)
{
    int rc;
    VPPX_ENTER(ctx);
    p.seed = ctx->rnd_seed;
    p.rand_offset = ctx->rnd_consumed;
    int64_t nh = 0;
    if ((rc = vppx_vpp_host(ctx, &p, 1, height, width, channels, l, r, g, g_occ, nullptr, &nh))) return rc;
    if (p.method == VPPX_METHOD_RND) {
        uint64_t draws = 0;
        if ((rc = vppx_vpp_last_draws(ctx, 1, &draws))) return rc;
        ctx->rnd_consumed += draws;
    }
    return (int)nh;
}

extern "C" int vppx_virtual_projection_scan_rnd(vppx_ctx *ctx, uint8_t *l, uint8_t *r, const float *g, int width,
                                                int height, int channels, int uniform_color, int wsize, int direction,
                                                float c, float c_occ, const uint8_t *g_occ, int discard_occluded,
                                                int interpolate)
{
    VppxVppParams p;
    vppx_vpp_params_default(&p);
    p.method = VPPX_METHOD_RND;
    p.uniform_color = uniform_color; p.wsize = wsize; p.direction = direction; p.c = c; p.c_occ = c_occ;
    p.discard_occluded = discard_occluded; p.interpolate = interpolate;
    return scan_common(ctx, p, l, r, g, width, height, channels, g_occ);
}

extern "C" int vppx_virtual_projection_scan_max_dist(vppx_ctx *ctx, uint8_t *l, uint8_t *r, const float *g, int width,
                                                     int height, int channels, int uniform_color, int wsize,
                                                     int wsize_agg_x, int wsize_agg_y, int direction, float c, float c_occ,
                                                     const uint8_t *g_occ, int discard_occluded, int interpolate)
{
    VppxVppParams p;
    vppx_vpp_params_default(&p);
    p.method = VPPX_METHOD_MAXDIST;
    p.uniform_color = uniform_color; p.wsize = wsize; p.wsize_agg_x = wsize_agg_x; p.wsize_agg_y = wsize_agg_y;
    p.direction = direction; p.c = c; p.c_occ = c_occ;
    p.discard_occluded = discard_occluded; p.interpolate = interpolate;
    return scan_common(ctx, p, l, r, g, width, height, channels, g_occ);
}

extern "C" int vppx_rand_stream(vppx_ctx *ctx, uint32_t seed, uint64_t offset, int64_t n, int32_t *out)
{
    int rc;
    VPPX_ENTER(ctx);
    if (n < 0 || (n > 0 && !out)) { vppx_set_error("vppx_rand_stream: bad arguments"); return VPPX_E_INVALID_ARG; }
    if (n == 0) return 0;
    void *d;
    if ((rc = ws_reserve(ctx, WS_STAGE_A, (size_t)n * sizeof(int32_t), &d))) return rc;
    if ((rc = vpp_launch_rand_stream(ctx, seed, offset, n, (int32_t *)d))) return rc;
    if ((rc = download(ctx, out, d, (size_t)n * sizeof(int32_t)))) return rc;
    VPPX_HIP(hipStreamSynchronize(ctx->stream));
    return 0;
}

static int vpp_rsgm_one(vppx_ctx *ctx, const HotCall &c)
{
    int rc;
    const VppxOccParams *const op = c.op;
    const VppxVppParams *const vp = &c.vp;
    const VppxRsgmParams *const rp = c.rp;
    const int B = c.B, H = c.H, W = c.W, C = c.C;
    const u8 *const left = c.left, *const right = c.right, *g_occ = c.g_occ;
    const float *const g = c.g;
    u8 *l_vpp = c.l_vpp, *r_vpp = c.r_vpp, *const conf_out = c.conf_out;
    const size_t nb = (size_t)B * H * W * C, np = (size_t)B * H * W;
    const bool piped = pipeline_applies(ctx);
    u8 *l_user = l_vpp, *r_user = r_vpp, *conf_user = conf_out;
    if ((piped || !l_vpp) && (rc = ws_get(ctx, WS_VPP_L, nb, &l_vpp))) return rc;
    if ((piped || !r_vpp) && (rc = ws_get(ctx, WS_VPP_R, nb, &r_vpp))) return rc;
    float *omap = nullptr;
    u8 *conf = conf_out;
    if (op) {
        if ((rc = ws_get(ctx, WS_OCC_OMAP, np, &omap))) return rc;
        if ((piped || !conf_out) && (rc = ws_get(ctx, WS_OCC_OUT, np, &conf))) return rc;
    }
    FrontGuard guard{ctx};
    ctx->n_pipe_copy = 0;
    if (piped) {
        ctx->pipe_call = true;
        if ((rc = front_begin(ctx))) return rc;
        ctx->occ_done_recorded = false;
        if (op && conf_user) ctx->pipe_copy[ctx->n_pipe_copy++] = {conf_user, conf, np, true};
        if (l_user) ctx->pipe_copy[ctx->n_pipe_copy++] = {l_user, l_vpp, nb, false};
        if (r_user) ctx->pipe_copy[ctx->n_pipe_copy++] = {r_user, r_vpp, nb, false};
    }
    {
        const int nvol_prev = (ctx->last_sum_nvol && ctx->last_sum_D == rp->dmax && ctx->last_sum_B == B) ? ctx->last_sum_nvol
                                                                                                          : (B >= VPPX_FUSED_MIN_FRAMES ? 4 : 8);
        const size_t sum_lds = rsgm_sum_lds_bytes(ctx, rp->dmax, nvol_prev), cu_lds = 160 * 1024;
        const size_t left_over = cu_lds > sum_lds + 512 ? cu_lds - sum_lds - 512 : 2048;
        const bool sum_fills_cu = rp->dmax == 256 && nvol_prev == 4 && ctx->knobs.sum_trap == 2 && !ctx->knobs.sum_general;
        ctx->front_lds_budget = (piped && !sum_fills_cu && left_over < 64 * 1024 && left_over >= 6 * 1024) ? left_over : 64 * 1024;
    }
    stage_begin(ctx);
    if (op) {
        if ((rc = occ_launch(ctx, B, H, W, g, op->rx, op->ry, op->l, op->g, op->th_conf, op->th_filter, omap, conf))) return rc;
        stage_mark(ctx, ST_OCC);
        g_occ = conf;
        if (piped && conf_user) {
            if (!ctx->ev_occ_done) VPPX_HIP(hipEventCreateWithFlags(&ctx->ev_occ_done, hipEventDisableTiming));
            VPPX_HIP(hipEventRecord(ctx->ev_occ_done, ctx->stream));
            ctx->occ_done_recorded = true;
        }
    }
    VPPX_HIP(hipMemcpyAsync(l_vpp, left, nb, hipMemcpyDeviceToDevice, ctx->stream));
    VPPX_HIP(hipMemcpyAsync(r_vpp, right, nb, hipMemcpyDeviceToDevice, ctx->stream));
    VppGeom vg = {B, H, W, C};
    const float *filled_g = nullptr;
    if (vp->use_bilateral_patch) {
        float *fg;
        if ((rc = ws_get(ctx, WS_FILLED_G, (size_t)B * H * W, &fg))) return rc;
        if ((rc = vpp_launch_bilateral_fill(ctx, *vp, vg, left, g, fg))) return rc;
        filled_g = fg;
    }
    if ((rc = vpp_launch(ctx, *vp, vg, l_vpp, r_vpp, g, g_occ, filled_g, nullptr, nullptr, right))) return rc;
    if (ctx->draws_dst && vp->method == VPPX_METHOD_RND)
        VPPX_HIP(hipMemcpy2DAsync(ctx->draws_dst, 8, ctx->ws[WS_FRAME_TOT].p, 16, 8, (size_t)B, hipMemcpyDeviceToDevice, ctx->stream));
    RsgmGeom rg;
    make_geom(B, H, W, C, rp->dmax, rg);
    return rsgm_core(ctx, *rp, rg, left, l_vpp, r_vpp, c.disp_out, c.validhints ? g : nullptr, c.validhints);
}

static int vpp_rsgm_entry(vppx_ctx *ctx, const HotCall &c);
static int scaled_call(vppx_ctx *ctx, const HotCall &c);
static int eval_call(vppx_ctx *ctx, const HotCall &c);
static int sampled_call(vppx_ctx *ctx, const HotCall &c);

static HotCall hot_call(HotCall::Layer layer, const VppxOccParams *op, const VppxVppParams *vp, const VppxRsgmParams *rp, int B, int H, int W,
                        int C, const uint8_t *left, const uint8_t *right)
{
    HotCall c;
    c.layer = layer;
    c.op = op;
    if (vp) c.vp = *vp;
    c.vp_null = !vp;
    c.rp = rp;
    c.B = B; c.H = H; c.W = W; c.C = C;
    c.left = left; c.right = right;
    return c;
}

int vppx_hot_call_internal(vppx_ctx *ctx, const HotCall &c)
{
    const int rc = c.layer == HotCall::SAMPLED ? sampled_call(ctx, c)
                 : c.layer == HotCall::EVAL    ? eval_call(ctx, c)
                 : c.layer == HotCall::SCALED  ? scaled_call(ctx, c)
                                               : vpp_rsgm_entry(ctx, c);
    ctx->inputs_ev = nullptr;
    return rc;
}

extern "C" int vppx_inputs_ready_event(vppx_ctx *ctx, void *hip_event)
{
    VPPX_ENTER(ctx);
    VPPX_PIPE_KEEP(ctx);
    ctx->inputs_ev = hip_event;
    return 0;
// ... 586 lines not shown
                                             const uint8_t *g_occ, const float *gt, const float *validgt, uint8_t *conf_out, uint8_t *l_vpp,
                                             uint8_t *r_vpp, float *disp_out, float *disp_small, VppxMetrics *metrics_out, float *errormap,
                                             float *hints_out, float *validhints_out)
{
    VPPX_ENTER(ctx);
    VPPX_PIPE_KEEP(ctx);
    HotCall c = hot_call(HotCall::SAMPLED, op, vp, rp, B, H, W, C, left, right);
    c.sp = sp; c.ep = ep; c.smp = smp;
    c.g_occ = g_occ;
    c.conf_out = conf_out; c.l_vpp = l_vpp; c.r_vpp = r_vpp; c.disp_out = disp_out; c.disp_small = disp_small;
    c.gt = gt; c.validgt = validgt; c.metrics_out = metrics_out; c.errormap = errormap;
    c.src = src; c.validsrc = validsrc; c.guided = guided; c.hints_out = hints_out; c.validhints_out = validhints_out;
    return vppx_hot_call_internal(ctx, c);
}

static int vpp_rsgm_parts(vppx_ctx *ctx, const HotCall &c)
{
    int rc;
    const VppxRsgmParams *const rp = c.rp;
    const int B = c.B, H = c.H, W = c.W, C = c.C;
    const bool validhints = c.validhints != nullptr;
    const int chunk_env = ctx->knobs.chunk;
    int q = 0;
    if (chunk_env > 0) {
        q = chunk_env;
    } else if (chunk_env < 0 && !ctx->is_child && B >= 16 && !validhints) {
        RsgmGeom g1;
        make_geom(1, H, W, C, rp->dmax, g1);
        u16 lut[256];
        int maxp2 = 0;
        p2_lut_host(*rp, lut, &maxp2);
        if (!ctx->vert3_broken && ctx->vert3_rest <= 0 && (ctx->vert3_probed || !ctx->capturing) && v3_probe_once(ctx) == 0 && !ctx->vert3_broken) {
            const int fpr = rsgm_vert3_frames_per_round(ctx, g1.Wp, g1.D);
            bool fused = false;
            if (fpr >= 8 && fpr < B) {
                g1.B = fpr;
                if ((rc = fused_layout_wanted(ctx, g1, maxp2, &fused))) return rc;
            }
            if (fused) q = fpr;
        }
    }
    if (validhints) {
        const int fb = guided_frames_per_part(ctx, H, W, C, rp->dmax);
        if (fb < B && (q <= 0 || q > fb)) q = fb;
    }
    ctx->last_parts = 1;
    if (q <= 0 || q >= B) return vpp_rsgm_one(ctx, c);
    ctx->last_parts = 0;
    void *const inputs_ev = ctx->inputs_ev;
    std::vector<int> plan;
    {
        const int k = B / q, r = B % q;
        if (chunk_env < 0 && !validhints && r > 0 && k >= 1 && 3 * ((r + k - 1) / k) <= q) {
            for (int i = 0; i < k; i++) plan.push_back(q + r / k + (i < r % k ? 1 : 0));
        } else {
            int left_over = B;
            while (left_over > 0) {
                int nb = left_over % q;
                if (nb == 0) nb = q;
                else if (nb < 8 && left_over > q && !validhints) nb += q;
                plan.push_back(nb);
                left_over -= nb;
            }
        }
    }
    int lo = 0;
    unsigned long long *const draws_base = ctx->draws_dst;
    struct DrawsRestore { vppx_ctx *c; unsigned long long *p; ~DrawsRestore() { c->draws_dst = p; } } draws_restore{ctx, draws_base};
    for (size_t pi = 0; pi < plan.size(); pi++) {
        const int nb = plan[pi];
        ctx->inputs_ev = inputs_ev;
        ctx->stage_append = lo > 0;
        ctx->draws_dst = draws_base ? draws_base + lo : nullptr;
        rc = vpp_rsgm_one(ctx, c.frames(lo, nb));
        ctx->stage_append = false;
        if (rc) return rc;
        ctx->last_parts++;
        lo += nb;
    }
    return 0;
}

extern "C" int vppx_last_call_parts(vppx_ctx *ctx) { return ctx ? ctx->last_parts : 0; }
extern "C" int vppx_we_last_pieces(vppx_ctx *ctx) { return ctx ? ctx->we_last_pieces : 0; }
extern "C" int vppx_wsum_last_pieces(vppx_ctx *ctx) { return ctx ? ctx->wsum_last_pieces : 0; }
extern "C" int vppx_wsum_default_route(int B, int Hp, int Wp, int dmax, int p2max, int nsimd)
{
    return rsgm_wsum_default(B, Hp, Wp, dmax, p2max, nsimd) ? 1 : 0;
}

static int vpp_rsgm_parts_eval(vppx_ctx *ctx, const HotCall &c)
{
    const int rc = vpp_rsgm_parts(ctx, c);
    if (rc || !c.metrics_out) return rc;
    return eval_launch(ctx, c, c.H, c.W, c.disp_out);
}

static int vpp_rsgm_entry(vppx_ctx *ctx, const HotCall &c)
{
    int rc;
    routes_reset(ctx);
    if (!ctx->front_routes_keep) front_routes_reset(ctx);
    ctx->front_routes_keep = false;
    const size_t front_base = ctx->front_routes.size();
    if ((rc = lockstep_check(ctx))) return rc;
    if (c.vp_null || !c.rp || !c.left || !c.right || !c.g || !c.disp_out) { vppx_set_error("vppx_vpp_rsgm: NULL argument"); return VPPX_E_INVALID_ARG; }
    const VppxRsgmParams *const rp = c.rp;
    const int B = c.B;
    if ((rc = check_frames(B, c.H, c.W, c.C))) return rc;
    if ((rc = check_vpp_params(c.vp))) return rc;
    if ((rc = check_rsgm_params(*rp))) return rc;
    if (ctx->inputs_ev && !pipeline_applies(ctx)) {
        VPPX_HIP(hipStreamWaitEvent(ctx->stream, (hipEvent_t)ctx->inputs_ev, 0));
        ctx->inputs_ev = nullptr;
    }
    const int nsub = (ctx->stage_timing || ctx->is_child) ? 1 : (B >= 2 * ctx->nsub ? ctx->nsub : 1);
    if (nsub <= 1 && ctx->graph_mode && !ctx->stage_timing) {
        vppx_ctx::GraphKey key;
        memset(&key, 0, sizeof(key));
        key.B = B; key.H = c.H; key.W = c.W; key.C = c.C; key.vp = c.vp; key.rp = *rp;
        key.ptr[0] = c.left; key.ptr[1] = c.right; key.ptr[2] = c.g; key.ptr[3] = c.g_occ; key.ptr[4] = c.l_vpp; key.ptr[5] = c.r_vpp;
        key.ptr[6] = c.disp_out; key.ptr[7] = c.conf_out; key.ptr[8] = c.validhints;
        key.has_op = c.op ? 1 : 0;
        if (c.op) key.op = *c.op;
        key.stream = (void *)ctx->stream;
        if (c.metrics_out) {
            key.eval_ptr[0] = c.gt; key.eval_ptr[1] = c.validgt; key.eval_ptr[2] = c.metrics_out; key.eval_ptr[3] = c.errormap;
            key.eval_scale[0] = c.gt_scale; key.eval_scale[1] = c.Hg; key.eval_scale[2] = c.Wg; key.eval_scale[3] = c.valid_is_u8;
        }
        key.ws_gen = ctx->ws_gen;
        const bool lut_ok = ctx->lut_valid && ctx->lut_p2min == rp->p2min && ctx->lut_gamma == rp->gamma && ctx->lut_alpha == rp->alpha;
        if (lut_ok && ctx->gexec && ctx->have_gkey && memcmp(&key, &ctx->gkey, sizeof(key)) == 0) {
            VPPX_HIP(hipGraphLaunch(ctx->gexec, ctx->stream));
            ctx->graph_replays++;
            ctx->routes = ctx->graph_routes;
            for (const std::string &r : ctx->graph_front_routes) front_route_note(ctx, "%s", r.c_str());
            return 0;
        }
        if (lut_ok && ctx->have_lastkey && memcmp(&key, &ctx->lastkey, sizeof(key)) == 0) {
            if (ctx->gexec) { (void)hipGraphExecDestroy(ctx->gexec); ctx->gexec = nullptr; ctx->have_gkey = false; }
            hipError_t e = hipStreamBeginCapture(ctx->stream, hipStreamCaptureModeThreadLocal);
            if (e == hipSuccess) {
                ctx->capturing = true;
                rc = vpp_rsgm_parts_eval(ctx, c);
                ctx->capturing = false;
                hipGraph_t graph = nullptr;
                e = hipStreamEndCapture(ctx->stream, &graph);
                if (rc != 0) {
                    if (graph) (void)hipGraphDestroy(graph);
                    (void)hipGetLastError();
                    ctx->have_lastkey = false;
                    return rc;
                }
                if (e == hipSuccess && graph) {
                    e = hipGraphInstantiate(&ctx->gexec, graph, nullptr, nullptr, 0);
                    (void)hipGraphDestroy(graph);
                    if (e == hipSuccess) {
                        ctx->gkey = key;
                        ctx->have_gkey = true;
                        ctx->graph_routes = ctx->routes;
                        ctx->graph_front_routes.assign(ctx->front_routes.begin() + front_base, ctx->front_routes.end());
                        ctx->graph_captures++;
                        VPPX_HIP(hipGraphLaunch(ctx->gexec, ctx->stream));
                        ctx->graph_replays++;
                        return 0;
                    }
// ... 494 lines not shown
    const void *vols[8];
    int nvol, eb;
    VPPX_HIP(hipEventRecord(e0, ctx->stream));
    for (int i = 0; i < iters; i++) {
        rc = run_aggregation(ctx, p, g, ctx->last_gl, ctx->last_cl, cr,
                             (const u16 *)ctx->ws[WS_P2LUT].p, maxp2, vols, &nvol, &eb, which);
        if (rc) return rc;
    }
    VPPX_HIP(hipEventRecord(e1, ctx->stream));
    VPPX_HIP(hipEventSynchronize(e1));
    float ms = 0.f;
    VPPX_HIP(hipEventElapsedTime(&ms, e0, e1));
    *ms_out = ms / (float)iters;
    (void)hipEventDestroy(e0);
    (void)hipEventDestroy(e1);
    return 0;
}

#ifdef VPPX_EXPERIMENT
extern "C" int vppx_exp_overlap(vppx_ctx *ctx, int mode, int iters, float *ms)
{
    int rc;
    VPPX_ENTER(ctx);
    if (!ctx->have_last || ctx->last_vert != 3 || iters <= 0 || !ms) { vppx_set_error("vppx_exp_overlap: call the fused path first"); return VPPX_E_INVALID_ARG; }
    const VppxRsgmParams &p = ctx->last_rp;
    u16 lut_h[256];
    int maxp2;
    p2_lut_host(p, lut_h, &maxp2);
    const int B = ctx->last_B, Hp = ctx->last_Hp, Wp = ctx->last_Wp, D = ctx->last_D;
    const size_t ncell = (size_t)B * Hp * Wp * D;
    void *scratch;
    if ((rc = ws_reserve(ctx, WS_DSI, ncell * 2, &scratch))) return rc;
    const void *vols[8] = {ctx->ws[WS_PATHS].p, (const u8 *)ctx->ws[WS_PATHS].p + ncell, ctx->ws[WS_SV].p, (const u8 *)ctx->ws[WS_SV].p + ncell};
    hipStream_t sa = ctx->stream, sb = ctx->stream2;
    hipEvent_t e0, e1, a0, a1, b0, b1, ej;
    for (hipEvent_t *e : {&e0, &e1, &a0, &a1, &b0, &b1, &ej}) VPPX_HIP(hipEventCreate(e));
    VPPX_HIP(hipStreamSynchronize(sa));
    VPPX_HIP(hipStreamSynchronize(sb));
    float tot[3] = {0, 0, 0};
    for (int i = 0; i < iters; i++) {
        VPPX_HIP(hipEventRecord(e0, sa));
        VPPX_HIP(hipStreamWaitEvent(sb, e0, 0));
        if (mode & 2) {
            hipStream_t keep = ctx->stream;
            ctx->stream = sb;
            VPPX_HIP(hipEventRecord(b0, sb));
            rc = rsgm_launch_paths(ctx, B, Hp, Wp, D, ctx->last_gl, ctx->last_cl, ctx->last_cr, nullptr, (const u16 *)ctx->ws[WS_P2LUT].p, p.p1, scratch, 1, 0x11);
            VPPX_HIP(hipEventRecord(b1, sb));
            ctx->stream = keep;
            if (rc) return rc;
        }
        if (mode & 1) {
            VPPX_HIP(hipEventRecord(a0, sa));
            rc = rsgm_launch_sum_wta_lr(ctx, B, Hp, Wp, D, vols, 4, 1, (float *)ctx->ws[WS_DISP_L0].p, (float *)ctx->ws[WS_DISP_R0].p, uniq_factor(p.uniqueness), 1, 24 + maxp2);
            VPPX_HIP(hipEventRecord(a1, sa));
            if (rc) return rc;
        }
        VPPX_HIP(hipEventRecord(ej, sb));
        VPPX_HIP(hipStreamWaitEvent(sa, ej, 0));
        VPPX_HIP(hipEventRecord(e1, sa));
        VPPX_HIP(hipEventSynchronize(e1));
        float t = 0.f;
        VPPX_HIP(hipEventElapsedTime(&t, e0, e1)); tot[0] += t;
        if (mode & 1) { VPPX_HIP(hipEventElapsedTime(&t, a0, a1)); tot[1] += t; }
        if (mode & 2) { VPPX_HIP(hipEventElapsedTime(&t, b0, b1)); tot[2] += t; }
    }
    for (int k = 0; k < 3; k++) ms[k] = tot[k] / (float)iters;
    for (hipEvent_t e : {e0, e1, a0, a1, b0, b1, ej}) (void)hipEventDestroy(e);
    return 0;
}
#endif

extern "C" int vppx_time_aggregate(vppx_ctx *ctx, int iters, float *ms_out) { return time_aggregation(ctx, iters, 0, ms_out); }
extern "C" int vppx_time_aggregate_part(vppx_ctx *ctx, int iters, int part, float *ms_out)
{
    if (part != 1 && part != 2) { vppx_set_error("part must be 1 or 2"); return VPPX_E_INVALID_ARG; }
    return time_aggregation(ctx, iters, part, ms_out);
}
extern "C" int vppx_agg_kernel_ms(vppx_ctx *ctx, int last_n, float *avg_ms, int *n_used)
{
    int rc;
    VPPX_ENTER(ctx);
    if (ctx->nsub > 1 && ctx->sub[0]) ctx = ctx->sub[0];
    if (last_n <= 0) { ctx->agg_calls = 0; if (n_used) *n_used = 0; if (avg_ms) *avg_ms = 0.f; return 0; }
    if (!avg_ms) return VPPX_E_INVALID_ARG;
    long n = ctx->agg_calls < last_n ? ctx->agg_calls : last_n;
    if (n > vppx_ctx::AGG_RING) n = vppx_ctx::AGG_RING;
    double tot = 0.0;
    for (long i = 0; i < n; i++) {
        const int slot = (int)((ctx->agg_calls - 1 - i) % vppx_ctx::AGG_RING);
        float t = 0.f;
        VPPX_HIP(hipEventSynchronize(ctx->agg_ev[1][slot]));
        VPPX_HIP(hipEventElapsedTime(&t, ctx->agg_ev[0][slot], ctx->agg_ev[1][slot]));
        tot += t;
    }
    *avg_ms = n > 0 ? (float)(tot / (double)n) : 0.f;
    if (n_used) *n_used = (int)n;
    return 0;
}
extern "C" int vppx_we_kernel_ms(vppx_ctx *ctx, int last_n, float *avg_ms, int *n_used)
{
    int rc;
    VPPX_ENTER(ctx);
    VPPX_PIPE_KEEP(ctx);
    if (ctx->nsub > 1 && ctx->sub[0]) ctx = ctx->sub[0];
    if (last_n <= 0) { ctx->we_calls = 0; if (n_used) *n_used = 0; if (avg_ms) *avg_ms = 0.f; return 0; }
    if (!avg_ms) return VPPX_E_INVALID_ARG;
    long n = ctx->we_calls < last_n ? ctx->we_calls : last_n;
    if (n > vppx_ctx::AGG_RING) n = vppx_ctx::AGG_RING;
    double tot = 0.0;
    for (long i = 0; i < n; i++) {
        const int slot = (int)((ctx->we_calls - 1 - i) % vppx_ctx::AGG_RING);
        float t = 0.f;
        VPPX_HIP(hipEventSynchronize(ctx->we_ev[1][slot]));
        VPPX_HIP(hipEventElapsedTime(&t, ctx->we_ev[0][slot], ctx->we_ev[1][slot]));
        tot += t;
    }
    *avg_ms = n > 0 ? (float)(tot / (double)n) : 0.f;
    if (n_used) *n_used = (int)n;
    (void)rc;
    return 0;
}
extern "C" int vppx_time_aggregate_frames(vppx_ctx *ctx)
{
    if (ctx && !ctx->have_last && ctx->sub[0] && ctx->sub[0]->have_last) ctx = ctx->sub[0];
    return (ctx && ctx->have_last) ? ctx->last_B : 0;
}
extern "C" int vppx_uses_vert(vppx_ctx *ctx)
{
    if (ctx && !ctx->have_last && ctx->sub[0] && ctx->sub[0]->have_last) ctx = ctx->sub[0];
    if (!ctx || !ctx->have_last) return 0;
    return ctx->last_vert;
}

static int check_viz_args(const char *name, int B, int H, int W, int dilation, bool all_pointers)
{
    if (!all_pointers) { vppx_set_error("%s: NULL argument", name); return VPPX_E_INVALID_ARG; }
    if (B < 1 || H < 1 || W < 1) { vppx_set_error("%s: bad shape (B %d, %d x %d)", name, B, H, W); return VPPX_E_INVALID_ARG; }
    if (dilation < 0) { vppx_set_error("%s: dilation %d (>= 0)", name, dilation); return VPPX_E_INVALID_ARG; }
    if (dilation > VIZ_MAX_DILATION) {
        vppx_set_error("%s: dilation %d is above this build's limit of %d", name, dilation, VIZ_MAX_DILATION);
        return VPPX_E_UNSUPPORTED;
    }
    return 0;
}

static int check_viz_scale(const char *name, double scale)
{
    if (!(scale > 0.0)) { vppx_set_error("%s: scale %g (> 0)", name, scale); return VPPX_E_INVALID_ARG; }
    return 0;
}

static int check_viz_which(const char *name, unsigned which)
{
    if (which == 0 || (which & ~(unsigned)VPPX_VIZ_ALL)) {
        vppx_set_error("%s: which 0x%x (one or more of the VPPX_VIZ_* bits)", name, which);
        return VPPX_E_INVALID_ARG;
    }
    return 0;
}

extern "C" int vppx_error_colors_dev(vppx_ctx *ctx, int B, int H, int W, const float *errors, const float *mask, double scale, int bgr,
                                     int dilation, uint8_t *out)
{
    VPPX_ENTER(ctx);
    VPPX_PIPE_KEEP(ctx);
    int rc;
    if ((rc = check_viz_args("vppx_error_colors_dev", B, H, W, dilation, errors && out))) return rc;
    if ((rc = check_viz_scale("vppx_error_colors_dev", scale))) return rc;
    return viz_launch_error_colors(ctx, B, H, W, errors, mask, scale, bgr, dilation, out);
}

extern "C" int vppx_error_colors_host(vppx_ctx *ctx, int B, int H, int W, const float *errors, const float *mask, double scale, int bgr,
                                      int dilation, uint8_t *out)
{
    VPPX_ENTER(ctx);
    int rc;
    if ((rc = check_viz_args("vppx_error_colors_host", B, H, W, dilation, errors && out))) return rc;
    if ((rc = check_viz_scale("vppx_error_colors_host", scale))) return rc;
    const size_t npx = (size_t)B * H * W;
    void *de, *dm = nullptr, *dout;
    if ((rc = upload(ctx, WS_STAGE_A, errors, npx * sizeof(float), &de))) return rc;
    if (mask && (rc = upload(ctx, WS_STAGE_B, mask, npx * sizeof(float), &dm))) return rc;
    if ((rc = ws_reserve(ctx, WS_VIZ_OUT, npx * 3, &dout))) return rc;
    if ((rc = viz_launch_error_colors(ctx, B, H, W, (const float *)de, (const float *)dm, scale, bgr, dilation, (u8 *)dout))) return rc;
    if ((rc = download(ctx, out, dout, npx * 3))) return rc;
    VPPX_HIP(hipStreamSynchronize(ctx->stream));
    return 0;
}
// ... 78 lines not shown
```

### vppstereo_amd/csrc/vppx_internal.h

```cpp
#pragma once
#include <hip/hip_runtime.h>
#include <stdint.h>
#include <stdio.h>
#include <string>
#include <vector>

#include "../../include/vppx.h"

typedef uint8_t u8;
typedef uint16_t u16;
typedef uint32_t u32;
typedef uint64_t u64;

void vppx_set_error(const char *fmt, ...);

#define VPPX_HIP(call)                                                                              \
    do {                                                                                            \
        hipError_t e_ = (call);                                                                     \
        if (e_ != hipSuccess) {                                                                     \
            vppx_set_error("%s failed: %s (%s:%d)", #call, hipGetErrorString(e_), __FILE__, __LINE__); \
            return VPPX_E_HIP;                                                                      \
        }                                                                                           \
    } while (0)

#define VPPX_CHECK_LAUNCH() VPPX_HIP(hipGetLastError())

struct DevGuard {
    int prev = -1;
    bool changed = false;
    explicit DevGuard(int dev)
    {
        if (hipGetDevice(&prev) != hipSuccess) prev = -1;
        if (prev != dev) changed = (hipSetDevice(dev) == hipSuccess);
    }
    ~DevGuard()
    {
        if (changed && prev >= 0) (void)hipSetDevice(prev);
    }
};

struct DevBuf {
    void *p = nullptr;
    size_t cap = 0;
};

enum WsSlot {
    WS_HINT_X = 0,
    WS_HINT_REC,
    WS_HINT_DENSE,
    WS_HINT_BITS,
    WS_RCNT,
    WS_FILLED_G,
    WS_GRAY_CTX,
    WS_RLIST,
    WS_LWORK,
    WS_LWORK_CNT,
    WS_ROW_COUNT,
    WS_ROW_DRAWS,
    WS_ROW_BASE,
    WS_FRAME_TOT,
    WS_HINT_RANGE,
    WS_RAND,
    WS_SEEDS,
    WS_VPP_L,
    WS_VPP_R,
    WS_VPP_LSRC,
    WS_OCC_ZERO,
    WS_GRAY_L,
    WS_GRAY_LV,
    WS_GRAY_RV,
    WS_CENSUS_L,
    WS_CENSUS_R,
    WS_GRAY_L2,
    WS_CENSUS_L2,
    WS_CENSUS_R2,
    WS_PATHS,
    WS_S,
    WS_SV,
    WS_VSTATE,
    WS_VMIN,
    WS_V3ERR,
    WS_WE_TRACE,
    WS_WE_HAND,
    WS_WSUM_HAND,
    WS_DSI,
    WS_GUIDED_MAP,
    WS_DISP_L0,
    WS_DISP_L1,
    WS_DISP_R0,
    WS_DISP_R1,
    WS_FD8,
    WS_SPK_ROOTS,
    WS_SPK_NROOTS,
    WS_ROW_ANY,
    WS_LABEL,
    WS_LCOUNT,
    WS_P2LUT,
    WS_STAGE_A,
    WS_STAGE_B,
    WS_STAGE_C,
    WS_STAGE_D,
    WS_STAGE_E,
    WS_STAGE_F,
    WS_OCC_OMAP,
    WS_OCC_OUT,
    WS_OCC_TMP,
    WS_NHINTS,
    WS_HANDOFF_H,
    WS_HANDOFF_V,
    WS_PNG_RAW,
    WS_PNG_OFFS,
    WS_PNG_STATUS,
    WS_SCALE_L0,
    WS_SCALE_R0,
    WS_SCALE_G0,
    WS_SCALE_V0,
    WS_SCALE_L1,
    WS_SCALE_R1,
    WS_SCALE_G1,
    WS_SCALE_V1,
    WS_SCALE_DSMALL,
    WS_SCALE_TAB,
    WS_SCALE_HOST_D,
    WS_METRICS_PART,
    WS_METRICS_OUT,
    WS_VIZ_PART,
    WS_VIZ_OUT,
    WS_VIZ_AUX,
    WS_SAMPLE_G0,
    WS_SAMPLE_V0,
    WS_SAMPLE_G1,
    WS_SAMPLE_V1,
    WS_NUM
};

#define VPPX_MAX_STAGES 96
#define VPPX_MAX_DEVICES 64

struct vppx_ctx {
    int device = 0;
    hipStream_t stream = nullptr;
    bool own_stream = false;
    bool legacy_stream = false;
    hipStream_t stream2 = nullptr;
    hipEvent_t ev_fork = nullptr, ev_join = nullptr;
    int nsub = 1;
    vppx_ctx *sub[4] = {nullptr, nullptr, nullptr, nullptr};
    hipEvent_t sub_done[4] = {nullptr, nullptr, nullptr, nullptr};
    bool is_child = false;
    struct Knobs {
        int chunk = -1;
        int sum_general = 0;
        int gw = 0;
        int maxdist = 0;
        int we_line = 0;
        int sum_gl8 = 0;
        int sum_trap = 2;
        int we_next = 1;
        int we_split = 1;
        int we_layer = 0;
        int we_mute = 0;
        int we_stale = 0;
        int fs_fail_submit = 0;
        int fs_fail_from = 0;
        int we_lq = -1;
        int wsum = -1;
        int wsum_cut = 0;
        int sum_blocks = 0;
        unsigned long long guided_part_bytes = 48ull << 30;
    } knobs;
    std::vector<std::string> routes;
    std::vector<std::string> graph_routes;
    std::vector<std::string> front_routes;
    std::vector<std::string> graph_front_routes;
    bool front_routes_keep = false;
    int use_vert = -1;
    int last_vert = 0;
    int last_parts = 1;
#ifdef VPPX_EXPERIMENT
    std::string exp_we_trace;
#endif
    unsigned we_serial = 0;
    void *we_hand_seen = nullptr;
    size_t we_hand_cap = 0;
    int we_hand_geom[3] = {0, 0, 0};
    int we_last_pieces = 1;
    void *wsum_hand_seen = nullptr;
    size_t wsum_hand_cap = 0;
    int wsum_last_pieces = 1;
    bool wsum_route = false;
    bool we_beside_vert = false;
    unsigned long long *draws_dst = nullptr;
    int last_sum_nvol = 0;
    int last_sum_D = 0, last_sum_B = 0;
    bool pipeline = false;
    bool front_active = false;
    bool pipe_call = false;
    bool have_agg_done = false;
    bool pipe_early = false;
    int pipe_parity = 0;
    bool pipe_mid = false;
    bool agg_done_recorded = false;
    const u8 *last_gl = nullptr;
    const u32 *last_cl = nullptr, *last_cr = nullptr;
    hipStream_t stream_front = nullptr, main_saved = nullptr;
    hipEvent_t ev_agg_done = nullptr, ev_front_done = nullptr, ev_inputs_auto = nullptr;
    void *inputs_ev = nullptr;
    struct PipeCopy { void *dst; const void *src; size_t bytes; bool early; } pipe_copy[3];
    int n_pipe_copy = 0;
    hipEvent_t ev_occ_done = nullptr;
    bool occ_done_recorded = false;
    size_t front_lds_budget = 64 * 1024;
    void *xbuf_last = nullptr;
    size_t xbuf_last_bytes = 0;
    bool xbuf_cleared = false;
    unsigned *vert3_err = nullptr;
    bool vert3_broken = false;
    int vert3_rest = 0;
    int vert3_backoff = 64;
    bool vert3_probed = false;
    long lockstep_failures = 0;
    unsigned lockstep_last_serial = 0;
    struct V3Caps {
        bool ok = false;
        int nxcd = 0, cus_per_xcd = 0;
        int blocks_per_cu[4] = {0, 0, 0, 0};
        int blocks_per_cu16[4] = {0, 0, 0, 0};
        int ppw = 0;
        int wall_khz = 100000;
        int timeout_ms = 250;
        unsigned spin_limit = 0;
        unsigned serial = 0;
        int last_ppw = 0;
        bool ignore_lost = false;
    } v3;
    DevBuf ws[WS_NUM];
    std::string devname;
    uint32_t rnd_seed = 1;
    uint64_t rnd_consumed = 0;
    int last_B = 0, last_Hp = 0, last_Wp = 0, last_D = 0;
    VppxRsgmParams last_rp;
    bool have_last = false;
    static const int AGG_RING = 64;
    hipEvent_t agg_ev[2][AGG_RING];
    bool agg_ev_created = false;
    long agg_calls = 0;
    hipEvent_t we_ev[2][AGG_RING];
    long we_calls = 0;
    u16 lut_host[256];
    bool lut_valid = false;
    int lut_p2min = 0, lut_gamma = 0, lut_maxp2 = 0;
    float lut_alpha = 0.f;
    struct GraphKey {
        int B, H, W, C;
        VppxVppParams vp;
        VppxRsgmParams rp;
        const void *ptr[9];
        const void *eval_ptr[4];
        int eval_scale[4];
        VppxOccParams op;
        int has_op;
        void *stream;
        unsigned long ws_gen;
    };
    bool graph_mode = false, capturing = false;
    bool have_gkey = false, have_lastkey = false;
    GraphKey gkey, lastkey;
    hipGraphExec_t gexec = nullptr;
    unsigned long ws_gen = 0;
    long graph_replays = 0, graph_captures = 0;
    bool stage_timing = false;
    bool stage_append = false;
    int n_stages = 0;
    hipEvent_t ev[VPPX_MAX_STAGES + 1];
    bool ev_created = false;
    int stage_id[VPPX_MAX_STAGES];
    size_t total_bytes = 0;
    std::vector<long long> png_offs_host;
    int scale_key[6] = {0, 0, 0, 0, 0, 0};
    const void *scale_tab_at = nullptr;
    int last_scale_set = -1, last_sample_set = -1;
    long scale_tab_builds = 0;
    int scale_parity = 0;
    hipEvent_t ev_scaled = nullptr;
    int sample_parity = 0;
    hipEvent_t ev_sampled = nullptr;
};

struct HotCall {
    enum Layer { PLAIN, SCALED, EVAL, SAMPLED };
    Layer layer = PLAIN;
    const VppxOccParams *op = nullptr;
    VppxVppParams vp = {};
    bool vp_null = false;
    const VppxRsgmParams *rp = nullptr;
    const VppxScaleParams *sp = nullptr;
    const VppxEvalParams *ep = nullptr;
    const VppxSampleParams *smp = nullptr;
    int B = 0, H = 0, W = 0, C = 0;
    const u8 *left = nullptr, *right = nullptr;
    const float *g = nullptr;
    const u8 *g_occ = nullptr;
    const float *validhints = nullptr;
    u8 *conf_out = nullptr, *l_vpp = nullptr, *r_vpp = nullptr;
    float *disp_out = nullptr, *disp_small = nullptr;
    const float *gt = nullptr;
    const void *validgt = nullptr;
    int valid_is_u8 = 0;
    VppxMetrics *metrics_out = nullptr;
    float *errormap = nullptr;
    int gt_scale = 1, Hg = 0, Wg = 0;
    const float *src = nullptr;
    const void *validsrc = nullptr;
    int vsrc_is_u8 = 0, guided = 0;
    float *hints_out = nullptr, *validhints_out = nullptr;

    HotCall frames(int lo, int nb) const
    {
        HotCall p = *this;
        const size_t px = (size_t)lo * H * W, gpx = (size_t)lo * Hg * Wg;
        auto at = [](auto *ptr, size_t n) { return ptr ? ptr + n : nullptr; };
        p.B = nb;
        p.vp.seed = vp.seed + (uint32_t)lo;
        p.left = at(left, px * C);
        p.right = at(right, px * C);
        p.g = at(g, px);
        p.g_occ = at(g_occ, px);
        p.validhints = at(validhints, px);
        p.conf_out = at(conf_out, px);
// ... 24 lines not shown
    int rc = ws_reserve(ctx, s, count * sizeof(T), &p);
    *out = (T *)p;
    return rc;
}

void route_note(vppx_ctx *ctx, const char *fmt, ...) __attribute__((format(printf, 2, 3)));
static inline void routes_reset(vppx_ctx *ctx) { ctx->routes.clear(); }
void front_route_note(vppx_ctx *ctx, const char *fmt, ...) __attribute__((format(printf, 2, 3)));
static inline void front_routes_reset(vppx_ctx *ctx) { ctx->front_routes.clear(); }

enum {
    ST_VPP_COMPACT = 0,
    ST_VPP_RAND,
    ST_VPP_APPLY,
    ST_PAD_GRAY,
    ST_CENSUS,
    ST_AGGREGATE,
    ST_SUM_WTA,
    ST_WTA_RIGHT,
    ST_MEDIAN_INTERP,
    ST_POST,
    ST_OCC,
    ST_COUNT
};
void stage_begin(vppx_ctx *ctx);
void stage_mark(vppx_ctx *ctx, int stage);

struct RsgmGeom {
    int B, H, W, C;
    int Hp, Wp;
    int pad_l, pad_r, pad_t, pad_b;
    int D;
};

int rsgm_launch_pad_gray(vppx_ctx *ctx, const RsgmGeom &g, const u8 *img, u8 *gray);
int rsgm_launch_pad_gray_n(vppx_ctx *ctx, const RsgmGeom &g, int n, const u8 *const *img, u8 *const *gray);
int rsgm_launch_to_nchw(vppx_ctx *ctx, int B, int H, int W, int C, int mult, const u8 *src, void *dst, int bf16);
int rsgm_launch_census(vppx_ctx *ctx, int B, int Hp, int Wp, const u8 *gray, u32 *census);
int rsgm_launch_pad_gray_census(vppx_ctx *ctx, const RsgmGeom &g, const u8 *left, const u8 *left_vpp, const u8 *right_vpp, u8 *gray_left,
                                u32 *census_l, u32 *census_r);
int rsgm_launch_census_n(vppx_ctx *ctx, int B, int Hp, int Wp, int n, const u8 *const *gray, u32 *const *census);
int rsgm_launch_cost(vppx_ctx *ctx, int B, int Hp, int Wp, int D, const u32 *cl, const u32 *cr, u16 *dsi);
int rsgm_launch_guided_rows(vppx_ctx *ctx, const RsgmGeom &g, const u32 *cl, const u32 *cr, const float *hints,
                            const float *valid, int *gmap, u16 *rows, u32 *count);
int rsgm_launch_paths(vppx_ctx *ctx, int B, int Hp, int Wp, int D, const u8 *gray, const u32 *cl, const u32 *cr,
                      const u16 *dsi, const u16 *p2lut, int p1, void *paths, int elem_bytes, int dir_mask,
                      const int *gmap = nullptr);
int rsgm_vert3_probe(vppx_ctx *ctx, u32 *scratch_dev, bool *ok);
bool rsgm_vert3_supported(int B, int Hp, int Wp, int D, int maxp2);
bool rsgm_vert3_fits(const vppx_ctx *ctx, int B, int Wp, int D);
int rsgm_vert3_frames_per_round(const vppx_ctx *ctx, int Wp, int D);
bool rsgm_vert3_wide(const vppx_ctx *ctx, int B, int Wp, int D);
size_t rsgm_vert3_xbuf_bytes(int B, int Wp, int D);
void rsgm_vert3_plan(const vppx_ctx *ctx, int B, int Wp, int D, int *whole_frames, bool *rest_underfilled);
int rsgm_launch_vert3_range(vppx_ctx *ctx, hipStream_t stream, int B_total, int f0, int nB, int Hp, int Wp, int D, const u8 *gray,
                            const u32 *cl, const u32 *cr, const u16 *p2lut, int p1, u8 *sv, u32 *xbuf, unsigned *err, unsigned *err_dev,
                            bool next_to_we);
int rsgm_launch_vert3(vppx_ctx *ctx, hipStream_t stream, int B, int Hp, int Wp, int D, const u8 *gray, const u32 *cl,
                      const u32 *cr, const u16 *p2lut, int p1, u8 *sv, u32 *xbuf, unsigned *err, unsigned *err_dev);
int rsgm_launch_void_if_lost(vppx_ctx *ctx, float *out, size_t n, const unsigned *err_dev, unsigned serial);
bool rsgm_vert_supported(int D, int maxp2);
size_t rsgm_vert_state_bytes(int B, int Wp, int D);
size_t rsgm_vert_min_elems(int B, int Wp);
int rsgm_launch_vert(vppx_ctx *ctx, hipStream_t stream, int B, int Hp, int Wp, int D, const u8 *gray, const u32 *cl,
                     const u32 *cr, const u16 *p2lut, int p1, u8 *sv, u8 *gst, u16 *gmin);
int rsgm_launch_sum_wta(vppx_ctx *ctx, int B, int Hp, int Wp, int D, const void *paths, int elem_bytes, u16 *S,
                        u16 *ST, float *disp_l, u32 factor_uniq, int do_subpixel);
int rsgm_launch_wta_right_t(vppx_ctx *ctx, int B, int Hp, int Wp, int D, const u16 *ST, float *disp, u32 factor_uniq);
int rsgm_paths_elem_bytes(int D, int maxp2);
size_t rsgm_sum_lds_bytes(const vppx_ctx *ctx, int D, int nvol);
bool rsgm_wsum_default(int B, int Hp, int Wp, int D, int maxp2, int nsimd);
bool rsgm_wsum_eligible(const vppx_ctx *ctx, int B, int Hp, int Wp, int D, int maxp2, int nsimd);
int rsgm_device_simds(vppx_ctx *ctx);
int rsgm_launch_wsum(vppx_ctx *ctx, int B, int Hp, int Wp, int D, const u8 *gray, const u32 *cl, const u32 *cr, const u16 *p2lut, int p1,
                     const void *vol_e, const void *vol_n3, const void *vol_s3, float *disp_l, float *disp_r, u32 fu);
int rsgm_launch_sum_wta_lr(vppx_ctx *ctx, int B, int Hp, int Wp, int D, const void *const *vols, int nvol, int elem_bytes,
                           float *disp_l, float *disp_r, u32 factor_uniq, int do_subpixel, int max_path_value);
int rsgm_launch_wta_left(vppx_ctx *ctx, int B, int Hp, int Wp, int D, const u16 *S, float *disp, u32 factor_uniq);
int rsgm_launch_subpixel(vppx_ctx *ctx, int B, int Hp, int Wp, int D, const u16 *S, float *disp);
int rsgm_launch_wta_right(vppx_ctx *ctx, int B, int Hp, int Wp, int D, const u16 *S, float *disp, u32 factor_uniq);
int rsgm_launch_median(vppx_ctx *ctx, int B, int Hp, int Wp, const float *src, float *dst);
int rsgm_launch_median_interp_clip(vppx_ctx *ctx, int B, int Hp, int Wp, const float *src_l, float *dst_l, const float *src_r,
                                   float *dst_r);
int rsgm_launch_post(vppx_ctx *ctx, const RsgmGeom &g, const float *dl_pad, const float *dr_pad, int subpixel, float *out);

struct VppGeom {
    int B, H, W, C;
};
int vpp_launch(vppx_ctx *ctx, const VppxVppParams &p, const VppGeom &g, u8 *l, u8 *r, const float *gmap,
               const u8 *occ, const float *filled_g, int64_t *n_hints_dev, const u32 *seeds_dev, const u8 *r_orig = nullptr);
int vpp_launch_bilateral_fill(vppx_ctx *ctx, const VppxVppParams &p, const VppGeom &g, const u8 *left, const float *gmap,
                              float *filled_out);
int vpp_launch_rand_stream(vppx_ctx *ctx, u32 seed, u64 offset, int64_t n, int32_t *out_dev);
u64 vpp_draws_upper_bound(const VppxVppParams &p, const VppGeom &g);

int handoff_psmnet_cost_volume(vppx_ctx *ctx, const void *fl, const void *fr, const float *hints, const float *valid, int B, int C,
                               int H4, int W4, int H, int W, int maxdisp, void *cost, int dtype);
int handoff_raft_corr_modulate(vppx_ctx *ctx, void *corr, const float *hints, const float *valid, int B, int H4, int W2, int W3, int H,
                               int W, int dtype);
int handoff_kitti_decode(vppx_ctx *ctx, const uint16_t *png, size_t n, float *disp, u8 *valid);
int handoff_pfm_decode(vppx_ctx *ctx, const u8 *raw, int H, int W, int channels, int little, float *out);
int handoff_subsample_hints(vppx_ctx *ctx, const float *hints, const float *valid, int B, int H, int W, int H4, int W4, float **hs,
                            float **vs, int raft);
int corr_pyramid(vppx_ctx *ctx, void *corr, const float *hints, const float *valid, int B, int H4, int W2, int W3, int H, int W,
                 int levels, void *pyr, int dtype);
int corr_lookup(vppx_ctx *ctx, const void *corr, const void *pyr, const float *coords_x, int64_t coords_frame_stride, int B, int H4,
                int W2, int W3, int levels, int radius, float *out, int dtype);
static inline int64_t corr_pyramid_offsets(int64_t N, int W3, int levels, int64_t *off)
{
    int64_t cells = 0;
    if (off) off[0] = 0;
    for (int i = 1; i < levels; i++) {
        if (off) off[i] = cells;
        cells += N * (int64_t)(W3 >> i);
    }
    return cells;
}

int readout_psm(vppx_ctx *ctx, const void *cost, int B, int D4, int H4, int W4, int D, int H, int W, int top, int left, int Hout,
                int Wout, float *out, int dtype);
int readout_raft_upsample(vppx_ctx *ctx, const void *flow, int64_t flow_frame_stride, const void *mask, int B, int C, int H4, int W4, int f,
                          int sign, int top, int left, int Hout, int Wout, float *out, int dtype);

__device__ __forceinline__ float modulation(float v, float h, float d, float two_w2)
{
    const float diff = __fsub_rn(d, h);
    const float e = expf(__fdiv_rn(-__fmul_rn(diff, diff), two_w2));
    return __fadd_rn(__fsub_rn(1.0f, v), __fmul_rn(__fmul_rn(v, 10.0f), e));
}

__device__ __forceinline__ float bf16_widen(u32 bits) { return __uint_as_float(bits << 16); }

__device__ __forceinline__ u32 bf16_rne(float f)
{
    const u32 u = __float_as_uint(f);
    if ((u & 0x7FFFFFFFu) > 0x7F800000u) return (u >> 16) | 0x0040u;
    return (u + 0x7FFFu + ((u >> 16) & 1u)) >> 16;
}

__device__ __forceinline__ u32 bf16_scale(u32 bits, float mod) { return bf16_rne(__fmul_rn(bf16_widen(bits), mod)); }
int handoff_png_decode(vppx_ctx *ctx, int n_files, const u8 *blob_dev, const long long *offs_dev, int H, int W, int C, u8 *zcat,
                       const long long *zoffs_dev, float scale, float *disp, u8 *valid, u8 *out_u8, int *status_dev);

struct ScaleFrontArgs {
    const u8 *l, *r;
    const float *g, *vh;
    u8 *ls, *rs;
    float *gs, *vhs;
    const int4 *ytab;
    const int4 *xtab;
    int B, H, W, C, h, w, s;
    float fs;
    long long n_img_threads;
};
int scale_launch_front(vppx_ctx *ctx, const ScaleFrontArgs &a);
int scale_launch_restore(vppx_ctx *ctx, int B, int h, int w, int Ho, int Wo, const float *src, float *out, const int *ry,
                         const int *rx, int iscale, int oscale);

#define METRICS_PARTIAL_BYTES 64
#define METRICS_MAX_BLOCKS 64
int metrics_blocks_per_frame(size_t npx);
int metrics_launch(vppx_ctx *ctx, int B, int Ho, int Wo, const float *disp, int Hg, int Wg, int gt_scale, const float *gt,
                   const void *valid, int valid_is_u8, void *partials, VppxMetrics *out, float *errormap);

int sample_launch(vppx_ctx *ctx, int B, size_t npx, const float *src, const void *vsrc, int vsrc_is_u8, float *hints, float *vhints,
                  const u32 *seeds_dev, u32 seed, u32 T);
u32 sample_threshold(double p);
// ... 14 lines not shown
```

### vppstereo_amd/engine.py

```python
import ctypes as C

from . import _lib


def _ptr(t):
    return C.c_void_p(t.data_ptr()) if t is not None else None


class Engine:

    def __init__(self, device=None):
        import torch
        if not torch.cuda.is_available():
            raise RuntimeError("vppstereo_amd.Engine needs an MI355X (no CPU fallback)")
        self.torch = torch
        self.device = torch.device("cuda", torch.cuda.current_device() if device is None else device)
        self.ctx = _lib.Context(self.device.index)
        self.lib = _lib.load()

    def _bind_stream(self):
        self.ctx.set_stream(self.torch.cuda.current_stream(self.device).cuda_stream)

    def _chk(self, t, dtype, ndim, name, shape=None):
        if t.device != self.device or t.dtype != dtype or t.dim() != ndim or not t.is_contiguous():
# ... 605 lines not shown
            offs[i + 1] = offs[i] + len(b)
        blob = torch.frombuffer(bytearray(b"".join(files)), dtype=torch.uint8).to(self.device)
        status = torch.empty((n,), dtype=torch.int32, device=self.device)
        disp = valid = out = None
        if want == "disp":
            disp = torch.empty((n, height, width), dtype=torch.float32, device=self.device)
            valid = torch.empty((n, height, width), dtype=torch.uint8, device=self.device)
        else:
            out = torch.empty((n, height, width, channels), dtype=torch.uint8, device=self.device)
        self._bind_stream()
        _lib.check(self.lib.vppx_png_decode_dev(self.ctx.handle, n, _ptr(blob), offs.ctypes.data_as(C.POINTER(C.c_int64)),
                                                int(height), int(width), int(channels), float(scale), _ptr(disp), _ptr(valid),
                                                _ptr(out), _ptr(status)))
        st = status.cpu().numpy()
        if st.any():
            bad = int(np.flatnonzero(st)[0])
            raise ValueError(f"png_decode: file {bad} rejected with status {int(st[bad])} (see include/vppx.h)")
        return (disp, valid) if want == "disp" else out

    def pfm_decode(self, raw_u8, height, width, channels=1, little_endian=True):
        torch = self.torch
        self._chk(raw_u8, torch.uint8, 1, "raw")
        if raw_u8.numel() != height * width * channels * 4:
            raise ValueError("payload size does not match height*width*channels*4")
        out = torch.empty((height, width, 3) if channels == 3 else (height, width), dtype=torch.float32, device=self.device)
        self._bind_stream()
        _lib.check(self.lib.vppx_pfm_decode_dev(self.ctx.handle, _ptr(raw_u8), int(height), int(width), int(channels),
                                                int(bool(little_endian)), _ptr(out)))
        return out

    def synchronize(self):
        self._bind_stream()
        self.ctx.synchronize()

    def status(self):
        self.ctx.status()

    def set_pipeline(self, enable=True):
        _lib.check(self.lib.vppx_set_pipeline(self.ctx.handle, int(bool(enable))))

    def set_graph_mode(self, enable=True):
        _lib.check(self.lib.vppx_set_graph_mode(self.ctx.handle, int(bool(enable))))

    def graph_replays(self):
        return int(self.lib.vppx_graph_replays(self.ctx.handle))

    def last_front_sets(self):
        a, b = C.c_int(-1), C.c_int(-1)
        _lib.check(self.lib.vppx_last_front_sets(self.ctx.handle, C.byref(a), C.byref(b)))
        return int(a.value), int(b.value)

    def scale_table_builds(self):
        return int(self.lib.vppx_scale_table_builds(self.ctx.handle))

    def time_aggregate(self, iters=10):
        ms = C.c_float()
        _lib.check(self.lib.vppx_time_aggregate(self.ctx.handle, int(iters), C.byref(ms)))
        return float(ms.value)

    def agg_kernel_ms(self, last_n):
        ms, n = C.c_float(0), C.c_int(0)
        _lib.check(self.lib.vppx_agg_kernel_ms(self.ctx.handle, int(last_n), C.byref(ms), C.byref(n)))
        return float(ms.value), int(n.value)

    def we_kernel_ms(self, last_n):
        ms, n = C.c_float(0), C.c_int(0)
        _lib.check(self.lib.vppx_we_kernel_ms(self.ctx.handle, int(last_n), C.byref(ms), C.byref(n)))
        return float(ms.value), int(n.value)

    def time_aggregate_frames(self):
        return int(self.lib.vppx_time_aggregate_frames(self.ctx.handle))

    def time_aggregate_part(self, part, iters=10):
        ms = C.c_float()
        _lib.check(self.lib.vppx_time_aggregate_part(self.ctx.handle, int(iters), int(part), C.byref(ms)))
        return float(ms.value)

    def uses_vert(self):
        return int(self.lib.vppx_uses_vert(self.ctx.handle))

    def last_call_parts(self):
        return int(self.lib.vppx_last_call_parts(self.ctx.handle))

    def we_last_pieces(self):
        return int(self.lib.vppx_we_last_pieces(self.ctx.handle))

    def wsum_last_pieces(self):
        return int(self.lib.vppx_wsum_last_pieces(self.ctx.handle))

    def last_routes(self):
        return _lib.last_routes(self.lib, self.ctx.handle)

    def last_front_routes(self):
        return _lib.last_front_routes(self.lib, self.ctx.handle)

    def fused_pixels_per_wave(self):
        return int(self.lib.vppx_fused_pixels_per_wave(self.ctx.handle))

    def batch_quantum(self, h, w, dmax=192):
        return int(self.lib.vppx_batch_quantum(self.ctx.handle, int(h), int(w), int(dmax)))

    def enable_stage_timing(self, on=True):
        _lib.check(self.lib.vppx_enable_stage_timing(self.ctx.handle, int(bool(on))))

    def stage_ms(self):
        arr = (C.c_float * 32)()
        n = _lib.check(self.lib.vppx_get_stage_ms(self.ctx.handle, arr, 32))
        return {self.lib.vppx_stage_name(i).decode(): float(arr[i]) for i in range(n)}
```

Measured before the change: 435,600.

## Fuse post-processing tail into one epilogue kernel and thin event timing

Folds several tail steps of the fused-vertical rSGM path into a single epilogue kernel: the edge-row interpolation, the void-if-lost NaN fill, the deferred pipeline output copies and the xbuf zeroing. This replaces multiple small kernel launches, memcpyAsyncs and a memset at the end of each call. It also records aggregation timing events only every seventh call instead of on every call, and double-buffers the VPP/occlusion workspaces by pipeline parity. The cost is more complex stream and clear-state bookkeeping, plus a risk of ordering bugs between the deferred copies and later frames.

```diff
diff --git a/include/vppx.h b/include/vppx.h
--- a/include/vppx.h
+++ b/include/vppx.h
@@ -323,6 +323,7 @@
 int vppx_fused_pixels_per_wave(vppx_ctx *ctx);
 int vppx_batch_quantum(vppx_ctx *ctx, int H, int W, int dmax);
 int vppx_last_call_parts(vppx_ctx *ctx);
+long vppx_epilogue_launches(vppx_ctx *ctx);
 int vppx_we_last_pieces(vppx_ctx *ctx);
 int vppx_wsum_last_pieces(vppx_ctx *ctx);
 int vppx_wsum_default_route(int B, int Hp, int Wp, int dmax, int p2max, int nsimd);
diff --git a/vppstereo_amd/_lib.py b/vppstereo_amd/_lib.py
--- a/vppstereo_amd/_lib.py
+++ b/vppstereo_amd/_lib.py
@@ -20,7 +20,7 @@
     "vppx_rand_stream", "vppx_rand_state", "vppx_rand_advance", "vppx_virtual_projection_scan_rnd", "vppx_virtual_projection_scan_max_dist", "vppx_vpp_host",
     "vppx_vpp_dev", "vppx_vpp_last_draws", "vppx_census5x5", "vppx_cost_census5x5_xyd", "vppx_aggregate", "vppx_aggregate_img", "vppx_match_wta",
     "vppx_match_wta_right", "vppx_subpixel_refine", "vppx_median3x3", "vppx_rsgm_host", "vppx_rsgm_dev",
-    "vppx_vpp_rsgm_dev", "vppx_rsgm_post_dev", "vppx_occ_vpp_rsgm_dev", "vppx_occ_vpp_rsgm_host", "vppx_inputs_ready_event", "vppx_u8_to_nchw_dev", "vppx_psmnet_cost_volume_dev", "vppx_raft_corr_modulate_dev", "vppx_kitti_disp_decode_dev", "vppx_png_decode_dev", "vppx_pfm_decode_dev", "vppx_occlusion_heuristic_host", "vppx_occlusion_heuristic_dev", "vppx_occlusion_heuristic_full_host", "vppx_occlusion_heuristic_full_dev", "vppx_set_graph_mode", "vppx_graph_replays", "vppx_time_aggregate", "vppx_agg_kernel_ms", "vppx_we_kernel_ms", "vppx_time_aggregate_frames", "vppx_time_aggregate_part", "vppx_uses_vert", "vppx_last_call_parts", "vppx_we_last_pieces", "vppx_wsum_last_pieces", "vppx_wsum_default_route", "vppx_last_routes", "vppx_last_front_routes", "vppx_fused_pixels_per_wave", "vppx_batch_quantum",
+    "vppx_vpp_rsgm_dev", "vppx_rsgm_post_dev", "vppx_occ_vpp_rsgm_dev", "vppx_occ_vpp_rsgm_host", "vppx_inputs_ready_event", "vppx_u8_to_nchw_dev", "vppx_psmnet_cost_volume_dev", "vppx_raft_corr_modulate_dev", "vppx_kitti_disp_decode_dev", "vppx_png_decode_dev", "vppx_pfm_decode_dev", "vppx_occlusion_heuristic_host", "vppx_occlusion_heuristic_dev", "vppx_occlusion_heuristic_full_host", "vppx_occlusion_heuristic_full_dev", "vppx_set_graph_mode", "vppx_graph_replays", "vppx_time_aggregate", "vppx_agg_kernel_ms", "vppx_we_kernel_ms", "vppx_time_aggregate_frames", "vppx_time_aggregate_part", "vppx_uses_vert", "vppx_last_call_parts", "vppx_epilogue_launches", "vppx_we_last_pieces", "vppx_wsum_last_pieces", "vppx_wsum_default_route", "vppx_last_routes", "vppx_last_front_routes", "vppx_fused_pixels_per_wave", "vppx_batch_quantum",
     "vppx_enable_stage_timing", "vppx_get_stage_ms", "vppx_stage_name",
     "vppx_fstream_create", "vppx_fstream_destroy", "vppx_fstream_push", "vppx_fstream_flush", "vppx_fstream_pop", "vppx_fstream_counts",
     "vppx_occ_vpp_rsgm_guided_dev", "vppx_occ_vpp_rsgm_guided_host", "vppx_fstream_push_guided",
@@ -200,6 +200,8 @@
         lib.vppx_time_aggregate_part.argtypes = [vp, i, i, C.POINTER(C.c_float)]
         lib.vppx_uses_vert.argtypes = [vp]
         lib.vppx_last_call_parts.argtypes = [vp]
+        lib.vppx_epilogue_launches.argtypes = [vp]
+        lib.vppx_epilogue_launches.restype = C.c_long
         lib.vppx_we_last_pieces.argtypes = [vp]
         lib.vppx_wsum_last_pieces.argtypes = [vp]
         lib.vppx_wsum_default_route.argtypes = [i, i, i, i, i, i]
diff --git a/vppstereo_amd/csrc/rsgm_kernels.hip b/vppstereo_amd/csrc/rsgm_kernels.hip
--- a/vppstereo_amd/csrc/rsgm_kernels.hip
+++ b/vppstereo_amd/csrc/rsgm_kernels.hip
@@ -2260,7 +2260,8 @@
         ++ctx->v3.serial;
         if (ctx->v3.serial == 0) ++ctx->v3.serial;
         const size_t xbytes = rsgm_vert3_xbuf_bytes(B_total, Wp, D);
-        if (!(ctx->xbuf_cleared && !ctx->capturing && ctx->xbuf_last == (void *)xbuf && ctx->xbuf_last_bytes >= xbytes && stream == ctx->stream))
+        if (!(ctx->xbuf_cleared && !ctx->capturing && ctx->xbuf_last == (void *)xbuf && ctx->xbuf_last_bytes >= xbytes && stream == ctx->stream &&
+              stream == ctx->xbuf_clear_stream))
             VPPX_HIP(hipMemsetAsync(xbuf, 0, xbytes, stream));
         ctx->xbuf_last = (void *)xbuf;
         ctx->xbuf_last_bytes = xbytes;
@@ -4189,19 +4190,19 @@
     __syncthreads();
     for (int x = threadIdx.x; x < W; x += 256) g[x] = res[x];
 }
-__global__ void __launch_bounds__(256) interp_bg_edge_rows_kernel(float *__restrict__ dm, const u8 *__restrict__ row_any, int H, int W)
+__device__ __forceinline__ void interp_bg_edge_rows_frame(float *__restrict__ g, const u8 *__restrict__ row_any, int H, int W)
 {
     __shared__ int s_first[4], s_last[4];
-    const int f = blockIdx.x, lane = threadIdx.x & 63, wv = threadIdx.x >> 6;
-    float *g = dm + (size_t)f * H * W;
+    const int lane = threadIdx.x & 63, wv = threadIdx.x >> 6;
     int first = 0x7FFFFFFF, last = -1;
     for (int v = threadIdx.x; v < H; v += 256)
-        if (row_any[(size_t)f * H + v]) { first = min(first, v); last = max(last, v); }
+        if (row_any[v]) { first = min(first, v); last = max(last, v); }
 #pragma unroll
     for (int off = 32; off >= 1; off >>= 1) {
         first = min(first, __shfl_xor(first, off));
         last = max(last, __shfl_xor(last, off));
     }
+    __syncthreads();
     if (lane == 0) s_first[wv] = first, s_last[wv] = last;
     __syncthreads();
     first = min(min(s_first[0], s_first[1]), min(s_first[2], s_first[3]));
@@ -4210,6 +4211,11 @@
     for (size_t i = threadIdx.x; i < (size_t)first * W; i += 256) g[i] = g[(size_t)first * W + i % W];
     for (size_t i = (size_t)(last + 1) * W + threadIdx.x; i < (size_t)H * W; i += 256) g[i] = g[(size_t)last * W + i % W];
 }
+__global__ void __launch_bounds__(256) interp_bg_edge_rows_kernel(float *__restrict__ dm, const u8 *__restrict__ row_any, int H, int W)
+{
+    const int f = blockIdx.x;
+    interp_bg_edge_rows_frame(dm + (size_t)f * H * W, row_any + (size_t)f * H, H, W);
+}
 
 __global__ void __launch_bounds__(256) void_if_lost_kernel(float *__restrict__ out, size_t n, const unsigned *__restrict__ err_dev,
                                                            unsigned serial)
@@ -4227,7 +4233,81 @@
     return 0;
 }
 
-int rsgm_launch_post(vppx_ctx *ctx, const RsgmGeom &g, const float *dl_pad, const float *dr_pad, int subpixel, float *out)
+typedef unsigned int epi_u32x4 __attribute__((ext_vector_type(4)));
+typedef unsigned int epi_u32x4_u __attribute__((ext_vector_type(4), aligned(1)));
+struct EpiArgs {
+    float *out;
+    const u8 *row_any;
+    int B, H, W;
+    const unsigned *err_dev;
+    unsigned serial;
+    int ncopy;
+    struct { u8 *dst; const u8 *src; size_t bytes; } copy[3];
+    u8 *xbuf;
+    size_t xbytes;
+};
+__global__ void __launch_bounds__(256) part_epilogue_kernel(EpiArgs a)
+{
+    const size_t tid = (size_t)blockIdx.x * 256 + threadIdx.x, nthr = (size_t)gridDim.x * 256;
+    const bool lost = __hip_atomic_load(a.err_dev, __ATOMIC_RELAXED, __HIP_MEMORY_SCOPE_AGENT) == a.serial;
+    if (lost) {
+        const float nan = __builtin_nanf("");
+        const size_t n = (size_t)a.B * a.H * a.W;
+        for (size_t i = tid; i < n; i += nthr) a.out[i] = nan;
+    } else {
+        for (int f = blockIdx.x; f < a.B; f += gridDim.x)
+            interp_bg_edge_rows_frame(a.out + (size_t)f * a.H * a.W, a.row_any + (size_t)f * a.H, a.H, a.W);
+    }
+    for (int c = 0; c < a.ncopy; c++) {
+        u8 *__restrict__ dst = a.copy[c].dst;
+        const u8 *__restrict__ src = a.copy[c].src;
+        const size_t n = a.copy[c].bytes;
+        size_t head = (size_t)(-(uintptr_t)dst & 15);
+        if (head > n) head = n;
+        const size_t nv = (n - head) / 16, tail0 = head + nv * 16;
+        for (size_t i = tid; i < nv; i += nthr) *(epi_u32x4 *)(dst + head + i * 16) = *(const epi_u32x4_u *)(src + head + i * 16);
+        if (tid < head) dst[tid] = src[tid];
+        if (tid < n - tail0) dst[tail0 + tid] = src[tail0 + tid];
+    }
+    if (a.xbytes) {
+        const size_t nv = a.xbytes / 16;
+        const epi_u32x4 z = {0u, 0u, 0u, 0u};
+        for (size_t i = tid; i < nv; i += nthr) ((epi_u32x4 *)a.xbuf)[i] = z;
+        if (tid < a.xbytes - nv * 16) a.xbuf[nv * 16 + tid] = 0;
+    }
+}
+
+int rsgm_launch_part_epilogue(vppx_ctx *ctx, const RsgmGeom &g, float *out, const unsigned *err_dev, unsigned serial,
+                              const vppx_ctx::PipeCopy *copies, int ncopy, void *xbuf, size_t xbytes)
+{
+    if (ncopy < 0 || ncopy > 3 || !ctx->ws[WS_ROW_ANY].p || ctx->ws[WS_ROW_ANY].cap < (size_t)g.B * g.H) {
+        vppx_set_error("part epilogue: bad arguments");
+        return VPPX_E_INVALID_ARG;
+    }
+    EpiArgs a;
+    a.out = out; a.row_any = (const u8 *)ctx->ws[WS_ROW_ANY].p;
+    a.B = g.B; a.H = g.H; a.W = g.W;
+    a.err_dev = err_dev; a.serial = serial;
+    a.ncopy = ncopy;
+    size_t most = xbytes;
+    for (int i = 0; i < 3; i++) {
+        a.copy[i].dst = i < ncopy ? (u8 *)copies[i].dst : nullptr;
+        a.copy[i].src = i < ncopy ? (const u8 *)copies[i].src : nullptr;
+        a.copy[i].bytes = i < ncopy ? copies[i].bytes : 0;
+        if (a.copy[i].bytes > most) most = a.copy[i].bytes;
+    }
+    a.xbuf = (u8 *)xbuf; a.xbytes = xbuf ? xbytes : 0;
+    size_t nblk = (most + 256 * 32 - 1) / (256 * 32);
+    if (nblk < (size_t)g.B) nblk = (size_t)g.B;
+    if (nblk > 1024) nblk = 1024;
+    if (nblk < 1) nblk = 1;
+    part_epilogue_kernel<<<(unsigned)nblk, 256, 0, ctx->stream>>>(a);
+    VPPX_CHECK_LAUNCH();
+    ctx->epilogue_launches++;
+    return 0;
+}
+
+int rsgm_launch_post(vppx_ctx *ctx, const RsgmGeom &g, const float *dl_pad, const float *dr_pad, int subpixel, float *out, bool edge_rows)
 {
     const size_t n = (size_t)g.B * g.H * g.W, npf = (size_t)g.H * g.W;
     if (g.W > 8192) { vppx_set_error("frame width %d > 8192 is not supported by the post-processing kernels", g.W); return VPPX_E_UNSUPPORTED; }
@@ -4261,7 +4341,9 @@
         speckle_apply_rows_kernel<32><<<dim3(g.H, g.B), 256, lds, ctx->stream>>>(fd8, label, size, dl_pad, out, row_any, g.H, g.W, g.Hp, g.Wp,
                                                                                 g.pad_t, g.pad_l, 0, 200, subpixel);
     VPPX_CHECK_LAUNCH();
-    interp_bg_edge_rows_kernel<<<g.B, 256, 0, ctx->stream>>>(out, row_any, g.H, g.W);
-    VPPX_CHECK_LAUNCH();
+    if (edge_rows) {
+        interp_bg_edge_rows_kernel<<<g.B, 256, 0, ctx->stream>>>(out, row_any, g.H, g.W);
+        VPPX_CHECK_LAUNCH();
+    }
     return 0;
 }
diff --git a/vppstereo_amd/csrc/vppx_api.hip b/vppstereo_amd/csrc/vppx_api.hip
--- a/vppstereo_amd/csrc/vppx_api.hip
+++ b/vppstereo_amd/csrc/vppx_api.hip
@@ -225,6 +225,7 @@
             }
             if (has("wsum")) ctx->knobs.wsum = 1;
             if (has("nowsum")) ctx->knobs.wsum = 0;
+            if (has("noepilogue")) ctx->knobs.epilogue = 0;
             {
                 const size_t wc = v.find("wsum_cut=");
                 if (wc != std::string::npos) ctx->knobs.wsum_cut = atoi(v.c_str() + wc + 9);
@@ -335,6 +336,7 @@
         if (rc) return rc;
         ctx->stream = (hipStream_t)hip_stream;
         ctx->legacy_stream = false;
+        ctx->xbuf_cleared = false;
     } else if (!ctx->own_stream) {
         VPPX_HIP(hipStreamCreateWithFlags(&ctx->stream, hipStreamNonBlocking));
         ctx->own_stream = true;
@@ -354,6 +356,7 @@
     if (rc) return rc;
     ctx->stream = nullptr;
     ctx->legacy_stream = true;
+    ctx->xbuf_cleared = false;
     return 0;
 }
 
@@ -709,7 +712,7 @@
         const int we_dirs = ctx->wsum_route ? 0x10 : 0x11;
         bool we_launched = false;
         auto launch_we = [&]() -> int {
-            const bool timed = !ctx->capturing;
+            const bool timed = !ctx->capturing && ctx->we_seq++ % vppx_ctx::MARK_EVERY == 0;
             if (timed && (rc = agg_events_create(ctx))) return rc;
             const int slot = (int)(ctx->we_calls % vppx_ctx::AGG_RING);
 #ifdef VPPX_EXPERIMENT
@@ -735,7 +738,7 @@
                 }
                 ctx->vert3_err[0] = 0;
             }
-            const bool timed = !ctx->capturing && st == ctx->stream;
+            const bool timed = !ctx->capturing && st == ctx->stream && ctx->agg_seq++ % vppx_ctx::MARK_EVERY == 0;
             if (timed && (rc = agg_events_create(ctx))) return rc;
             const int slot = (int)(ctx->agg_calls % vppx_ctx::AGG_RING);
             if (timed) VPPX_HIP(hipEventRecord(ctx->agg_ev[0][slot], st));
@@ -877,9 +880,15 @@
     ctx->stream = ctx->main_saved;
     ctx->front_active = false;
     VPPX_HIP(hipEventRecord(ctx->ev_front_done, front));
+    if (ctx->epi_defer) {
+        for (int i = 0; i < ctx->n_pipe_copy; i++) ctx->epi_copy[i] = ctx->pipe_copy[i];
+        ctx->n_epi_copy = ctx->n_pipe_copy;
+        ctx->n_pipe_copy = 0;
+    }
     if (ctx->xbuf_last && !ctx->xbuf_cleared && ctx->xbuf_last == ctx->ws[WS_VSTATE].p) {
         VPPX_HIP(hipMemsetAsync(ctx->xbuf_last, 0, ctx->xbuf_last_bytes, ctx->stream));
         ctx->xbuf_cleared = true;
+        ctx->xbuf_clear_stream = ctx->stream;
     }
     if (ctx->occ_done_recorded) {
         bool any = false;
@@ -911,6 +920,8 @@
         }
         ctx->pipe_call = false;
         ctx->n_pipe_copy = 0;
+        ctx->n_epi_copy = 0;
+        ctx->epi_defer = false;
         ctx->occ_done_recorded = false;
     }
 };
@@ -934,6 +945,16 @@
             if ((rc = fused_layout_wanted(ctx, g, mp2, &fused))) return rc;
         }
         ctx->pipe_early = ctx->pipe_call && g.B < 8 && !fused;
+    }
+    ctx->epi_defer = false;
+    ctx->n_epi_copy = 0;
+    if (ctx->front_active && ctx->n_pipe_copy > 0 && ctx->knobs.epilogue && !(hints && validhints)) {
+        u16 lut_tmp[256];
+        int mp2 = 0;
+        bool fused = false;
+        p2_lut_host(p, lut_tmp, &mp2);
+        if ((rc = fused_layout_wanted(ctx, g, mp2, &fused))) return rc;
+        ctx->epi_defer = fused;
     }
     if ((rc = ws_get(ctx, alt ? WS_GRAY_L2 : WS_GRAY_L, npp, &gl))) return rc;
     if ((rc = ws_get(ctx, alt ? WS_CENSUS_L2 : WS_CENSUS_L, npp, &cl))) return rc;
@@ -995,9 +1016,25 @@
     { float *t = dl0; dl0 = dl1; dl1 = t; t = dr0; dr0 = dr1; dr1 = t; }
 
     const size_t np = (size_t)g.B * g.H * g.W;
-    if ((rc = rsgm_launch_post(ctx, g, dl0, dr0, p.subpixel, disp_out))) return rc;
-    if (ctx->last_vert == 3 && ctx->ws[WS_V3ERR].p &&
-        (rc = rsgm_launch_void_if_lost(ctx, disp_out, np, (const unsigned *)ctx->ws[WS_V3ERR].p, ctx->v3.serial))) return rc;
+    const bool fused_now = ctx->last_vert == 3 && !(hints && validhints) && ctx->ws[WS_V3ERR].p;
+    const bool epilogue = fused_now && ctx->knobs.epilogue && !ctx->stage_timing && !ctx->is_child;
+    if ((rc = rsgm_launch_post(ctx, g, dl0, dr0, p.subpixel, disp_out, !epilogue))) return rc;
+    if (epilogue) {
+        const bool clear = !ctx->capturing && ctx->xbuf_last && !ctx->xbuf_cleared && ctx->xbuf_last == ctx->ws[WS_VSTATE].p &&
+                           ctx->xbuf_last_bytes <= ctx->ws[WS_VSTATE].cap;
+        if ((rc = rsgm_launch_part_epilogue(ctx, g, disp_out, (const unsigned *)ctx->ws[WS_V3ERR].p, ctx->v3.serial, ctx->epi_copy,
+                                            ctx->n_epi_copy, clear ? ctx->xbuf_last : nullptr, clear ? ctx->xbuf_last_bytes : 0))) return rc;
+        if (clear) {
+            ctx->xbuf_cleared = true;
+            ctx->xbuf_clear_stream = ctx->stream;
+        }
+    } else {
+        if (ctx->last_vert == 3 && ctx->ws[WS_V3ERR].p &&
+            (rc = rsgm_launch_void_if_lost(ctx, disp_out, np, (const unsigned *)ctx->ws[WS_V3ERR].p, ctx->v3.serial))) return rc;
+        for (int i = 0; i < ctx->n_epi_copy; i++)
+            VPPX_HIP(hipMemcpyAsync(ctx->epi_copy[i].dst, ctx->epi_copy[i].src, ctx->epi_copy[i].bytes, hipMemcpyDeviceToDevice, ctx->stream));
+    }
+    ctx->n_epi_copy = 0;
     stage_mark(ctx, ST_POST);
     return 0;
 }
@@ -1305,14 +1342,15 @@
     u8 *l_vpp = c.l_vpp, *r_vpp = c.r_vpp, *const conf_out = c.conf_out;
     const size_t nb = (size_t)B * H * W * C, np = (size_t)B * H * W;
     const bool piped = pipeline_applies(ctx);
+    const bool alt = piped && (ctx->pipe_parity & 1);
     u8 *l_user = l_vpp, *r_user = r_vpp, *conf_user = conf_out;
-    if ((piped || !l_vpp) && (rc = ws_get(ctx, WS_VPP_L, nb, &l_vpp))) return rc;
-    if ((piped || !r_vpp) && (rc = ws_get(ctx, WS_VPP_R, nb, &r_vpp))) return rc;
+    if ((piped || !l_vpp) && (rc = ws_get(ctx, alt ? WS_VPP_L2 : WS_VPP_L, nb, &l_vpp))) return rc;
+    if ((piped || !r_vpp) && (rc = ws_get(ctx, alt ? WS_VPP_R2 : WS_VPP_R, nb, &r_vpp))) return rc;
     float *omap = nullptr;
     u8 *conf = conf_out;
     if (op) {
         if ((rc = ws_get(ctx, WS_OCC_OMAP, np, &omap))) return rc;
-        if ((piped || !conf_out) && (rc = ws_get(ctx, WS_OCC_OUT, np, &conf))) return rc;
+        if ((piped || !conf_out) && (rc = ws_get(ctx, alt ? WS_OCC_OUT2 : WS_OCC_OUT, np, &conf))) return rc;
     }
     FrontGuard guard{ctx};
     ctx->n_pipe_copy = 0;
@@ -2065,6 +2103,7 @@
 }
 
 extern "C" int vppx_last_call_parts(vppx_ctx *ctx) { return ctx ? ctx->last_parts : 0; }
+extern "C" long vppx_epilogue_launches(vppx_ctx *ctx) { return ctx ? ctx->epilogue_launches : 0; }
 extern "C" int vppx_we_last_pieces(vppx_ctx *ctx) { return ctx ? ctx->we_last_pieces : 0; }
 extern "C" int vppx_wsum_last_pieces(vppx_ctx *ctx) { return ctx ? ctx->wsum_last_pieces : 0; }
 extern "C" int vppx_wsum_default_route(int B, int Hp, int Wp, int dmax, int p2max, int nsimd)
@@ -2725,7 +2764,7 @@
     int rc;
     VPPX_ENTER(ctx);
     if (ctx->nsub > 1 && ctx->sub[0]) ctx = ctx->sub[0];
-    if (last_n <= 0) { ctx->agg_calls = 0; if (n_used) *n_used = 0; if (avg_ms) *avg_ms = 0.f; return 0; }
+    if (last_n <= 0) { ctx->agg_calls = 0; ctx->agg_seq = 0; if (n_used) *n_used = 0; if (avg_ms) *avg_ms = 0.f; return 0; }
     if (!avg_ms) return VPPX_E_INVALID_ARG;
     long n = ctx->agg_calls < last_n ? ctx->agg_calls : last_n;
     if (n > vppx_ctx::AGG_RING) n = vppx_ctx::AGG_RING;
@@ -2747,7 +2786,7 @@
     VPPX_ENTER(ctx);
     VPPX_PIPE_KEEP(ctx);
     if (ctx->nsub > 1 && ctx->sub[0]) ctx = ctx->sub[0];
-    if (last_n <= 0) { ctx->we_calls = 0; if (n_used) *n_used = 0; if (avg_ms) *avg_ms = 0.f; return 0; }
+    if (last_n <= 0) { ctx->we_calls = 0; ctx->we_seq = 0; if (n_used) *n_used = 0; if (avg_ms) *avg_ms = 0.f; return 0; }
     if (!avg_ms) return VPPX_E_INVALID_ARG;
     long n = ctx->we_calls < last_n ? ctx->we_calls : last_n;
     if (n > vppx_ctx::AGG_RING) n = vppx_ctx::AGG_RING;
diff --git a/vppstereo_amd/csrc/vppx_internal.h b/vppstereo_amd/csrc/vppx_internal.h
--- a/vppstereo_amd/csrc/vppx_internal.h
+++ b/vppstereo_amd/csrc/vppx_internal.h
@@ -65,6 +65,9 @@
     WS_VPP_L,
     WS_VPP_R,
     WS_VPP_LSRC,
+    WS_VPP_L2,
+    WS_VPP_R2,
+    WS_OCC_OUT2,
     WS_OCC_ZERO,
     WS_GRAY_L,
     WS_GRAY_LV,
@@ -165,6 +168,7 @@
         int fs_fail_from = 0;
         int we_lq = -1;
         int wsum = -1;
+        int epilogue = 1;
         int wsum_cut = 0;
         int sum_blocks = 0;
         unsigned long long guided_part_bytes = 48ull << 30;
@@ -208,12 +212,17 @@
     void *inputs_ev = nullptr;
     struct PipeCopy { void *dst; const void *src; size_t bytes; bool early; } pipe_copy[3];
     int n_pipe_copy = 0;
+    bool epi_defer = false;
+    PipeCopy epi_copy[3];
+    int n_epi_copy = 0;
+    long epilogue_launches = 0;
     hipEvent_t ev_occ_done = nullptr;
     bool occ_done_recorded = false;
     size_t front_lds_budget = 64 * 1024;
     void *xbuf_last = nullptr;
     size_t xbuf_last_bytes = 0;
     bool xbuf_cleared = false;
+    hipStream_t xbuf_clear_stream = nullptr;
     unsigned *vert3_err = nullptr;
     bool vert3_broken = false;
     int vert3_rest = 0;
@@ -245,6 +254,8 @@
     hipEvent_t agg_ev[2][AGG_RING];
     bool agg_ev_created = false;
     long agg_calls = 0;
+    static const int MARK_EVERY = 7;
+    long agg_seq = 0, we_seq = 0;
     hipEvent_t we_ev[2][AGG_RING];
     long we_calls = 0;
     u16 lut_host[256];
@@ -435,7 +446,9 @@
 int rsgm_launch_median(vppx_ctx *ctx, int B, int Hp, int Wp, const float *src, float *dst);
 int rsgm_launch_median_interp_clip(vppx_ctx *ctx, int B, int Hp, int Wp, const float *src_l, float *dst_l, const float *src_r,
                                    float *dst_r);
-int rsgm_launch_post(vppx_ctx *ctx, const RsgmGeom &g, const float *dl_pad, const float *dr_pad, int subpixel, float *out);
+int rsgm_launch_post(vppx_ctx *ctx, const RsgmGeom &g, const float *dl_pad, const float *dr_pad, int subpixel, float *out, bool edge_rows = true);
+int rsgm_launch_part_epilogue(vppx_ctx *ctx, const RsgmGeom &g, float *out, const unsigned *err_dev, unsigned serial,
+                              const vppx_ctx::PipeCopy *copies, int ncopy, void *xbuf, size_t xbytes);
 
 struct VppGeom {
     int B, H, W, C;
diff --git a/vppstereo_amd/engine.py b/vppstereo_amd/engine.py
--- a/vppstereo_amd/engine.py
+++ b/vppstereo_amd/engine.py
@@ -711,6 +711,9 @@
     def last_call_parts(self):
         return int(self.lib.vppx_last_call_parts(self.ctx.handle))
 
+    def epilogue_launches(self):
+        return int(self.lib.vppx_epilogue_launches(self.ctx.handle))
+
     def we_last_pieces(self):
         return int(self.lib.vppx_we_last_pieces(self.ctx.handle))
 
```

Result: no change. 437,200 (median of 6 runs) (+0.4%).
